# AlbertoEsc/PyFaceAnalysis

Measured on AMD Instinct MI355X. Metric: 128x128 sub-images/sec through 11L HiGSFA net, higher is better.
Workload: dtype f32; 1 GPU; configs[1]: U11L-128 (11-layer net, trained random-init weights), 4096 synthetic 128x128 sub-images per GPU per step, float32 input resident in HBM, first 20 slow features out; rows_per_gpu=4096, global_rows=4096, plan=fused, parallelism=row-shard x1

## Files before the change

### pyfaceanalysis_amd/build.py

```python
from __future__ import annotations

import os
import subprocess
import sys

HERE = os.path.dirname(os.path.abspath(__file__))
CSRC = os.path.join(HERE, "csrc")
LIB = os.path.join(HERE, "libhigsfa.so")
SOURCES = ["hg_tree.cpp", "hg_capi.cpp", "hg_hostpack.cpp", "hg_resample.cpp", "hg_normalize.cpp", "hg_normalize.hip", "hg_generic.hip", "hg_fused_plan.cpp", "hg_fused_call.cpp", "hg_fused.hip", "hg_fused_sum.hip", "hg_fused_front.hip", "hg_fused_igsfa.hip", "hg_fused_prod.hip", "hg_fused_tail.hip",
           "hg_gauss.hip", "hg_extract.hip", "hg_resample.hip", "hg_cascade.hip", "hg_eyes.hip", "hg_estimate.hip", "hg_train.hip"]
HEADERS = ["hg_common.hpp", os.path.join("..", "..", "include", "higsfa.h")]
HOST_ONLY = {"hg_hostpack.cpp": [], "hg_resample.cpp": ["-ffp-contract=off"], "hg_normalize.cpp": ["-ffp-contract=off"]}
HIPCC = os.environ.get("HIPCC", "/opt/rocm/bin/hipcc")
CXX = os.environ.get("CXX", "g++")
FLAGS = ["-O3", "-std=c++17", "-fPIC", "--offload-arch=gfx950", "-Wall", "-Wno-unused-result"]
if os.environ.get("HIGSFA_CXXFLAGS"):
    FLAGS += os.environ["HIGSFA_CXXFLAGS"].split()
if os.environ.get("HIGSFA_DIAG"):
    FLAGS.append("-DHIGSFA_DIAG")


def _newer(a, b):
    return (not os.path.exists(b)) or os.path.getmtime(a) > os.path.getmtime(b)


def _header_paths():
    hdr = [os.path.join(CSRC, h) for h in HEADERS]
    return hdr + [os.path.join(CSRC, h) for h in os.listdir(CSRC) if h.endswith((".hpp", ".h", ".inc"))]


def is_stale():
    if not os.path.exists(LIB):
        return True
    hdr = _header_paths()
    for src in SOURCES:
        sp, op = os.path.join(CSRC, src), os.path.join(CSRC, "_obj", src + ".o")
        if _newer(sp, op) or any(_newer(h, op) for h in hdr) or _newer(op, LIB):
            return True
    return False


def oracle_is_stale(oracle_dir):
    pairs = (("ref_c.c", "libref_c.so"), ("fast_cpu.c", "libfast_cpu.so"), ("fast_cpu_pow.c", "libfast_cpu.so"))
    return any(os.path.exists(os.path.join(oracle_dir, c)) and _newer(os.path.join(oracle_dir, c), os.path.join(oracle_dir, so))
               for c, so in pairs)


def build(force=False, verbose=False):
    objdir = os.path.join(CSRC, "_obj")
    os.makedirs(objdir, exist_ok=True)
    hdr_paths = [os.path.join(CSRC, h) for h in HEADERS]
    hdr_paths += [os.path.join(CSRC, h) for h in os.listdir(CSRC) if h.endswith((".hpp", ".h", ".inc"))]
    objs, relink = [], force or not os.path.exists(LIB)
    procs = []
    for src in SOURCES:
        sp = os.path.join(CSRC, src)
        op = os.path.join(objdir, src + ".o")
        objs.append(op)
        if force or _newer(sp, op) or any(_newer(h, op) for h in hdr_paths):
            if src in HOST_ONLY:
                cmd = [CXX, "-O3", "-std=c++17", "-fPIC", "-Wall"] + HOST_ONLY[src] + ["-c", sp, "-o", op]
            else:
                cmd = [HIPCC] + FLAGS + (["-x", "hip"] if src.endswith(".hip") else []) + ["-c", sp, "-o", op]
            if verbose:
                print(" ".join(cmd), flush=True)
            procs.append((src, subprocess.Popen(cmd, stdout=subprocess.PIPE, stderr=subprocess.STDOUT)))
            relink = True
    for src, p in procs:
        out, _ = p.communicate()
        if p.returncode != 0:
            raise RuntimeError("hipcc failed on %s:\n%s" % (src, out.decode(errors="replace")))
        if verbose and out:
            print(out.decode(errors="replace"))
    if relink:
        cmd = [HIPCC, "-shared", "-fPIC", "--offload-arch=gfx950", "-o", LIB] + objs + ["-L/opt/rocm/lib", "-lrocsolver", "-lrocblas"]
        if verbose:
            print(" ".join(cmd), flush=True)
        r = subprocess.run(cmd, stdout=subprocess.PIPE, stderr=subprocess.STDOUT)
        if r.returncode != 0:
            raise RuntimeError("link failed:\n%s" % r.stdout.decode(errors="replace"))
    return LIB


if __name__ == "__main__":
    print(build(force="--force" in sys.argv, verbose=True))
```

### pyfaceanalysis_amd/csrc/hg_fused.hip

```cpp
#include <hip/hip_runtime.h>

#include <algorithm>
#include <cmath>
#include <cstdlib>
#include <map>
#include <sstream>
#include <tuple>

#include "hg_fused_dev.hpp"

namespace hg {

namespace {

using namespace fused;

#ifndef HG_A_PINGPONG
#define HG_A_PINGPONG 1
#endif
#ifdef HIGSFA_DIAG
#define HG_HOT(blk) ((P.whatif & 1) ? ((blk) & 1) : (blk))
#else
#define HG_HOT(blk) (blk)
#endif
// ... 374 lines not shown
                            }
                    }
                }
            }
        }
        if (rem1) {
#pragma unroll
            for (int t = 0; t < T; ++t) add_rem4(z[t], d4[t]);
        }
        if (!P.has_exp) {
#pragma unroll
            for (int t = 0; t < T; ++t)
                if (tile[t] < P.n_tiles) P.out[((size_t)tile[t] * P.nb_out + node * P.mto + w) * 64 + lane] = z[t];
            return;
        }
        for (int fi = 0; fi < nf; ++fi) {
            const int fk = (P.funcp >> (4 * fi)) & 15;
            const float ex = P.expo[fi];
#pragma unroll
            for (int t = 0; t < T; ++t) smem[((fi * mt1n + w) * T + t) * 64 + lane] = apply_func_uniform(fk, ex, z[t]);
        }
    } else if (!P.has_exp) {
        return;
    }
    __syncthreads();
    if (w >= mt2n) return;
#pragma unroll
    for (int t = 0; t < T; ++t) d4[t] = f32x4{0.f, 0.f, 0.f, 0.f};
    f32x4 y[T];
    {
        const f32x4 bb = *(const f32x4*)(bnode + (mt1n + w) * 16);
#pragma unroll
        for (int t = 0; t < T; ++t) y[t] = bb;
    }
#pragma unroll
    for (int k = 0; k < KB; ++k) {
        if (k >= k2n) continue;
        const int mt1 = k / nf, fi = k - mt1 * nf;
        const int nk = (P.nk2p[mt1] >> (4 * fi)) & 15;
        f32x4 e[T];
#pragma unroll
        for (int t = 0; t < T; ++t) e[t] = smem[((fi * mt1n + mt1) * T + t) * 64 + lane];
        if (REM && rem2) {
#pragma unroll
            for (int r = 0; r < 4; ++r)
                if (r < nk) {
#pragma unroll
                    for (int t = 0; t < T; ++t) d4[t] = MFMA4(a2[k][r], e[t][r], d4[t]);
                }
        } else if (nk == 4) {
#pragma unroll
            for (int r = 0; r < 4; ++r)
#pragma unroll
                for (int t = 0; t < T; ++t) y[t] = MFMA16(a2[k][r], e[t][r], y[t]);
        } else {
#pragma unroll
            for (int r = 0; r < 4; ++r)
                if (r < nk) {
#pragma unroll
                    for (int t = 0; t < T; ++t) y[t] = MFMA16(a2[k][r], e[t][r], y[t]);
                }
        }
    }
    if (rem2) {
#pragma unroll
        for (int t = 0; t < T; ++t) add_rem4(y[t], d4[t]);
    }
    if (REM && P.pack_base > 0) {
        if (rem2) {
            const int slot = __builtin_amdgcn_readfirstlane(P.pack_slot[node]);
#pragma unroll
            for (int t = 0; t < T; ++t)
                if (tile[t] < P.n_tiles) *packed_slot_ptr(P, tile[t], slot, lane) = y[t][0];
        } else {
#pragma unroll
            for (int t = 0; t < T; ++t)
                if (tile[t] < P.n_tiles) P.out[((size_t)tile[t] * P.nb_out + node * (mt2n - 1) + w) * 64 + lane] = y[t];
        }
        return;
    }
#pragma unroll
    for (int t = 0; t < T; ++t)
        if (tile[t] < P.n_tiles) P.out[((size_t)tile[t] * P.nb_out + node * P.mto + w) * 64 + lane] = y[t];
}

template <typename YT>
__global__ void k_unpack(const float* __restrict__ act, int nb, const int32_t* __restrict__ col_base, YT* __restrict__ y,
                         int64_t ldy, int64_t n, int cols) {
    int64_t total = n * cols;
    for (int64_t idx = (int64_t)blockIdx.x * blockDim.x + threadIdx.x; idx < total; idx += (int64_t)gridDim.x * blockDim.x) {
        int64_t row = idx / cols;
        int c = (int)(idx - row * cols);
        int64_t tile = row >> 4;
        int jj = (int)(row & 15);
        y[row * ldy + c] = (YT)act[tile * nb * 256 + col_base[c] + jj * 4];
    }
}


template <int MT1, int MT2>
StageFn pick_stage_t(int T) {
    if (T == 2) return k_stage<MT1, MT2, 2>;
    return k_stage<MT1, MT2, 1>;
}
template <int MT1>
StageFn pick_stage_m2(int mt2, int T) {
    switch (mt2) {
        case 1: return pick_stage_t<MT1, 1>(T);
        case 2: return pick_stage_t<MT1, 2>(T);
        case 3: return pick_stage_t<MT1, 3>(T);
        default: return pick_stage_t<MT1, 4>(T);
    }
}
StageFn pick_stage(int mt1, int mt2, int T, bool rem = false, int kbf = 0, bool fs = false, int pk = -1) {
    if (pk >= 0) {
        if (pk == 1 && kbf == 3 && T == 2 && rem && mt1 == 3 && mt2 == 3) return fs ? (StageFn)k_stage<3, 3, 2, false, true, 3, true, 1> : (StageFn)k_stage<3, 3, 2, false, true, 3, false, 1>;
        if (pk == 1 && kbf == 3 && T == 2 && rem && mt1 == 2 && mt2 == 2) return (StageFn)k_stage<2, 2, 2, false, true, 3, false, 1>;
        return nullptr;
    }
    if (fs) {
        if (kbf == 3 && T == 2 && rem && mt1 == 3 && mt2 == 3) return (StageFn)k_stage<3, 3, 2, false, true, 3, true>;
        if (kbf == 4 && T == 2 && !rem && mt1 == 3 && mt2 == 3) return (StageFn)k_stage<3, 3, 2, false, false, 4, true>;
        if (kbf == 0 && !rem && mt1 == 4 && mt2 == 4) return T == 2 ? (StageFn)k_stage<4, 4, 2, false, false, 0, true> : (StageFn)k_stage<4, 4, 1, false, false, 0, true>;
    }
    if (kbf == 4 && T == 2) {
        if (rem && mt1 == 3 && mt2 == 3) return (StageFn)k_stage<3, 3, 2, false, true, 4>;
        if (rem && mt1 == 2 && mt2 == 2) return (StageFn)k_stage<2, 2, 2, false, true, 4>;
        if (!rem && mt1 == 3 && mt2 == 3) return (StageFn)k_stage<3, 3, 2, false, false, 4>;
        if (!rem && mt1 == 2 && mt2 == 2) return (StageFn)k_stage<2, 2, 2, false, false, 4>;
    }
    if (kbf == 3 && T == 2) {
        if (rem && mt1 == 3 && mt2 == 3) return (StageFn)k_stage<3, 3, 2, false, true, 3>;
        if (rem && mt1 == 2 && mt2 == 2) return (StageFn)k_stage<2, 2, 2, false, true, 3>;
    }
    if (rem) {
        if (mt1 == 3 && mt2 == 3) return T == 2 ? (StageFn)k_stage<3, 3, 2, false, true> : (StageFn)k_stage<3, 3, 1, false, true>;
        if (mt1 == 2 && mt2 == 2) return T == 2 ? (StageFn)k_stage<2, 2, 2, false, true> : (StageFn)k_stage<2, 2, 1, false, true>;
    }
    switch (mt1) {
        case 1: return pick_stage_m2<1>(mt2, T);
        case 2: return pick_stage_m2<2>(mt2, T);
        case 3: return pick_stage_m2<3>(mt2, T);
        default: return pick_stage_m2<4>(mt2, T);
    }
}



struct StageDev {
    DevBuf afrag, bias, kb1tab, chunks, runs, piece, koff, kmean, kcol, gcol, etab, pack_slot;
    DevBuf fold_frag, fold_bias;
    DevBuf fold_last;
    DevBuf pair_kids, kb1tab_pre, bias_pre;
};
struct SubRunDev {
    DevBuf nodes[kMaxTail], tab[kMaxTail];
};

struct WorkQueue {
    DevBuf ctr;
    uint32_t base = 0;
};

constexpr int kMaxLanes = 2;
struct Lane {
    DevBuf bufA, bufB;
    int64_t cap_rows = 0;
    WorkQueue wq_front, wq_direct, wq_direct_wg;
    int32_t* err_host = nullptr;
    int32_t* err_dev = nullptr;
    std::vector<CallStep> steps;
};

class FusedExecutor : public Executor {
public:
    explicit FusedExecutor(std::unique_ptr<const FusedPlan> plan) : plan_(std::move(plan)) {}

    int plan_kind() const override { return HG_PLAN_FUSED; }
    int n_stages() const override { return (int)plan_->stages.size() + 1; }
    std::string stage_name(int i) const override {
        if (i == 1 && plan_->fuse01 && !plan_->opt.fold01)
            return plan_->stages[i].name + "  [link 0 -> 1 stays as it is: switched off (HIGSFA_NO_FOLD01)]";
        if (i == 1 && plan_->fold01 && !plan_->opt.fold01_pack)
            return plan_->stages[i].name + "  [the link's one-row k-steps stay as they are: switched off (HIGSFA_NO_FOLD01_PACK)]";
        if (i < (int)plan_->stages.size() && plan_->stages[i].sum_in && !plan_->opt.pair)
            return plan_->stages[i].name + "; unpaired: switched off (HIGSFA_NO_PAIR)";
        if (i < (int)plan_->stages.size()) return plan_->stages[i].name;
        return plan_->tail_begin >= 0 ? std::string("row-major y written by the top-of-hierarchy launch (no unpack pass)")
                                      : std::string("fused unpack (fragment order -> row-major y)");
    }
    std::string describe() const override {
        std::ostringstream os;
        os << "plan: FUSED (fragment-order activations, v_mfma_f32_16x16x4_f32)\n";
        for (int i = 0; i < n_stages(); ++i) os << "  [" << i << "] " << stage_name(i) << "\n";
        return os.str();
    }
    int64_t weight_bytes() const override {
        int64_t t = 0;
        for (auto& s : plan_->stages) t += (int64_t)(s.afrag.size() + s.bias.size()) * 4;
        return t;
    }
    int64_t padded_flops_per_row() const override { return plan_->padded_flops_given; }
    int64_t workspace_bytes() const override {
        int64_t t = 0;
        for (int l = 0; l < n_lanes_; ++l) t += (int64_t)(lanes_[l].bufA.bytes + lanes_[l].bufB.bytes);
        return t;
    }

    void to_device() override {
        dev_.resize(plan_->stages.size());
        for (size_t si = 0; si < dev_.size(); ++si) {
            const HostStage& s = plan_->stages[si];
            StageDev& d = dev_[si];
            if (plan_->fold01 && si < 2) {
                const size_t first = si == 0 ? 0 : (size_t)s.kb1 * s.mt1, count = si == 0 ? (size_t)s.kb1 * s.mt1 : (size_t)s.node_blocks - first;
                std::vector<float> part((size_t)s.n_nodes * count * 256);
                for (int ni = 0; ni < s.n_nodes; ++ni)
                    std::copy_n(s.afrag.data() + ((size_t)ni * s.node_blocks + first) * 256, count * 256, part.data() + (size_t)ni * count * 256);
                const bool variant = plan_->fold01_pack && si == 0;
                if (variant) d.afrag.upload(s.fold_a1.data(), s.fold_a1.size() * 4);
                else d.afrag.upload(part.data(), part.size() * 4);
                if (si == 1) {
                    d.fold_frag.upload(s.fold_frag.data(), s.fold_frag.size() * 4);
                    d.fold_bias.upload(s.fold_bias.data(), s.fold_bias.size() * 4);
                    if (plan_->fold01_pack) d.fold_last.upload(s.fold_last.data(), s.fold_last.size() * 4);
                }
            } else {
                d.afrag.upload(s.afrag.data(), s.afrag.size() * 4);
            }
            if (plan_->fold01_pack && si == 0) d.bias.upload(s.fold_b1.data(), s.fold_b1.size() * 4);
            else d.bias.upload(s.bias.data(), s.bias.size() * 4);
            if (!s.kb1tab.empty()) d.kb1tab.upload(s.kb1tab.data(), s.kb1tab.size() * 4);
            if (!s.gcol.empty()) d.gcol.upload(s.gcol.data(), s.gcol.size() * 4);
            if (!s.etab.empty()) d.etab.upload(s.etab.data(), s.etab.size() * 4);
            if (!s.pack_slot.empty()) d.pack_slot.upload(s.pack_slot.data(), s.pack_slot.size() * 4);
            if (!s.pair_kids.empty()) {
                d.pair_kids.upload(s.pair_kids.data(), s.pair_kids.size() * 4);
                d.kb1tab_pre.upload(s.kb1tab_pre.data(), s.kb1tab_pre.size() * 4);
                d.bias_pre.upload(s.bias_pre.data(), s.bias_pre.size() * 4);
            }
            if (!s.chunks.empty()) {
                d.chunks.upload(s.chunks.data(), s.chunks.size() * sizeof(DChunk));
                d.runs.upload(s.runs.data(), s.runs.size() * sizeof(DRun));
                d.piece.upload(s.piece_col.data(), s.piece_col.size() * 4);
                d.koff.upload(s.koff.data(), s.koff.size() * 4);
                d.kmean.upload(s.kmean.data(), s.kmean.size() * 4);
                if (!s.kcol.empty()) d.kcol.upload(s.kcol.data(), s.kcol.size() * 4);
            }
        }
        sub_dev_.resize(plan_->sub_runs.size());
        for (size_t ri = 0; ri < sub_dev_.size(); ++ri) {
            const SubRun& r = plan_->sub_runs[ri];
            for (int k = 0; k < r.len; ++k) {
                sub_dev_[ri].nodes[k].upload(r.nodes[k].data(), r.nodes[k].size() * 4);
                if (k > 0) sub_dev_[ri].tab[k].upload(r.tab[k].data(), r.tab[k].size() * 4);
            }
        }
        d_col_base_.upload(plan_->col_base.data(), plan_->col_base.size() * 4);
        d_col_of_.upload(plan_->col_of.data(), plan_->col_of.size() * 4);
        int dev = 0;
        hipDeviceProp_t prop;
        if (hipGetDevice(&dev) == hipSuccess && hipGetDeviceProperties(&prop, dev) == hipSuccess && prop.multiProcessorCount > 0)
            n_cus_ = prop.multiProcessorCount;
    }

    void reserve(int64_t rows) override {
        for (int l = 0; l < n_lanes_; ++l) reserve_lane(lanes_[l], rows);
    }

    bool set_lanes(int n) override {
        if (n < 1 || n > kMaxLanes) return false;
        for (int l = n; l < n_lanes_; ++l) release_lane(lanes_[l]);
        for (int l = n_lanes_; l < n; ++l) reserve_lane(lanes_[l], lanes_[0].cap_rows);
        n_lanes_ = n;
        return true;
    }
    int lanes() const override { return n_lanes_; }

    void run(const void* x, int x_dtype, int64_t n, int64_t ldx, void* y, int y_dtype, int64_t y_cols, int64_t ldy,
             hipStream_t st, hipEvent_t* ev) override {
        run_in(lanes_[0], x, x_dtype, n, ldx, y, y_dtype, y_cols, ldy, st, ev);
    }
    void run_lane(int lane, const void* x, int x_dtype, int64_t n, int64_t ldx, void* y, int y_dtype, int64_t y_cols, int64_t ldy,
                  hipStream_t st) override {
        if (lane < 0 || lane >= n_lanes_) fail(HG_ERR_ARG, "lane %d outside 0..%d", lane, n_lanes_ - 1);
        run_in(lanes_[lane], x, x_dtype, n, ldx, y, y_dtype, y_cols, ldy, st, nullptr);
    }

    void run_in(Lane& L, const void* x, int x_dtype, int64_t n, int64_t ldx, void* y, int y_dtype, int64_t y_cols, int64_t ldy,
                hipStream_t st, hipEvent_t* ev) {
        check_device_error();
        if (dev_.size() != plan_->stages.size()) fail(HG_ERR_STATE, "fused: the plan is not on a device");
        if (n > L.cap_rows) {
            if (n_lanes_ > 1) HG_HIP(hipStreamSynchronize(st));
            reserve_lane(L, n);
        }
        run_range(L, x, x_dtype, n, ldx, y, y_dtype, y_cols, ldy, st, ev);
    }

    void run_range(Lane& L, const void* x, int x_dtype, int64_t n, int64_t ldx, void* y, int y_dtype, int64_t y_cols, int64_t ldy,
                   hipStream_t st, hipEvent_t* ev) {
        const int n_tiles = (int)((n + 15) / 16);
        FrontInput fi;
        fi.vec4_ok = rows_vec4(x, ldx, x_dtype);
        fi.x_dtype = x_dtype;
        fi.ldx = ldx;
        plan_call(*plan_, n_tiles, fi, L.steps);
        int e = 0;
        auto record = [&](int k) {
            if (ev)
                for (int i = 0; i < k; ++i) HG_HIP(hipEventRecord(ev[e++], st));
        };
        record(1);
        f32x4* cur = (f32x4*)L.bufA.p;
        f32x4* nxt = (f32x4*)L.bufB.p;
        for (const CallStep& step : L.steps) {
            const int si = step.stage;
            if (step.route == Route::Top) {
                debug_line(step, 0, 1);
                launch_top(si, cur, n_tiles, y, y_dtype, y_cols, ldy, n, st);
                record(step.covered + 1);
                HG_HIP(hipGetLastError());
                return;
            }
            if (step.route == Route::Subtree) {
                debug_line(step, 0, 1);
                launch_subtrees(plan_->sub_runs[step.sub_run], sub_dev_[step.sub_run], cur, nxt, n_tiles, st);
                std::swap(cur, nxt);
                record(step.covered);
                continue;
            }
            const HostStage& s = plan_->stages[si];
            const StageDev& d = dev_[si];
            StageParams P = stage_params(s, d, cur, nxt, n_tiles);
            switch (step.route) {
                case Route::Gather:
                    debug_line(step, 0, 1);
                    launch_im2frag(x, x_dtype, ldx, n, n_tiles, s.nb_out, (const int32_t*)d.gcol.p, nxt, step.sh.vec4 ? 1 : 0, (unsigned)step_blocks(step, 1), st);
                    break;
                case Route::IgSweep:
                case Route::IgSplit: launch_igsfa(step, s, P, st); break;
                case Route::Front01d:
                case Route::Front01p: launch_front_pair(L, step, s, d, P, x, x_dtype, ldx, n, n_tiles, cur, st); break;
                case Route::Front0p:
                case Route::Front0: launch_front(step, s, d, P, x, x_dtype, ldx, n, st); break;
                case Route::ProdSweep: launch_prod(step, s, d, P, st); break;
                case Route::Splitm: launch_splitm(step, s, P, st); break;
                default:
                    if (step.in_summed) {
                        P.kb1tab = (const int2*)d.kb1tab_pre.p;
                        P.bias = (const float*)d.bias_pre.p;
                        P.kb1 = step.sh.kb1;
                        P.n_kids = step.sh.n_kids;
                        P.nb_in = s.n_nodes * s.mt1;
                    }
                    if (step.route == Route::SumPair) launch_stage_pair(step, s, plan_->stages[si + 1], dev_[si + 1], P, st);
                    else launch_stage(step, s, P, st);
            }
            if (step.covered == 1) std::swap(cur, nxt);
            record(step.covered);
        }
        launch_unpack(cur, n, y, y_dtype, y_cols, ldy, st);
        record(1);
        HG_HIP(hipGetLastError());
    }

    void release() override {
        for (Lane& L : lanes_) release_lane(L);
        n_lanes_ = 1;
        d_col_base_.free();
        d_col_of_.free();
        sub_dev_.clear();
        dev_.clear();
    }

private:
    void reserve_lane(Lane& L, int64_t rows) {
        int64_t tiles = (rows + 15) / 16;
        size_t need = (size_t)tiles * plan_->max_nb * 1024;
        L.bufA.alloc(need);
        L.bufB.alloc(need);
        L.cap_rows = std::max(L.cap_rows, tiles * 16);
        L.steps.reserve(plan_->stages.size());
    }
    void release_lane(Lane& L) {
        L.bufA.free();
        L.bufB.free();
        L.wq_front.ctr.free();
        L.wq_direct.ctr.free();
        L.wq_direct_wg.ctr.free();
        L.wq_front.base = L.wq_direct.base = L.wq_direct_wg.base = 0;
        if (L.err_host) (void)hipHostFree(L.err_host);
        L.err_host = nullptr;
        L.err_dev = nullptr;
        L.cap_rows = 0;
    }

    int resident_blocks(StageFn fn, int threads, size_t lds) {
        set_lds_limit(fn, lds);
        auto key = std::make_tuple((const void*)fn, threads, lds);
        auto it = occ_.find(key);
        if (it != occ_.end()) return it->second;
        int nb = 0;
        if (hipOccupancyMaxActiveBlocksPerMultiprocessor(&nb, (const void*)fn, threads, lds) != hipSuccess || nb < 1) nb = 1;
        occ_[key] = nb;
        return nb;
    }

    uint32_t* work_counters(WorkQueue& q, int n, hipStream_t st) {
        const size_t need = (size_t)n * 64;
        if (q.ctr.bytes < need) {
            q.ctr.alloc(std::max<size_t>(need, 64 * 1024));
            HG_HIP(hipMemsetD32Async((hipDeviceptr_t)q.ctr.p, (int)plan_->opt.wq_start, q.ctr.bytes / 4, st));
            q.base = plan_->opt.wq_start;
        }
        return (uint32_t*)q.ctr.p;
    }

    int32_t* device_error_word(Lane& L) {
        if (!L.err_host) {
            HG_HIP(hipHostMalloc((void**)&L.err_host, 64, hipHostMallocMapped));
            *L.err_host = 0;
            HG_HIP(hipHostGetDevicePointer((void**)&L.err_dev, L.err_host, 0));
        }
        return L.err_dev;
    }
    void check_errors() override { check_device_error(); }
    void check_device_error() {
        for (const Lane& L : lanes_)
            if (L.err_host && *(volatile int32_t*)L.err_host != 0)
                fail(HG_ERR_DEVICE, "fused: a bounded poll in a persistent kernel ran out (code %d); the features of that call are invalid", (int)*L.err_host);
    }

    void set_lds_limit(StageFn fn, size_t bytes) {
        if (bytes <= 64 * 1024) return;
        if (bytes > 160 * 1024) fail(HG_ERR_FORMAT, "fused: a node needs %zu bytes of LDS (> 160 KiB)", bytes);
        auto it = lds_set_.find((const void*)fn);
        if (it != lds_set_.end() && it->second >= bytes) return;
        HG_HIP(hipFuncSetAttribute((const void*)fn, hipFuncAttributeMaxDynamicSharedMemorySize, (int)(160 * 1024)));
        lds_set_[(const void*)fn] = 160 * 1024;
    }

    StageParams stage_params(const HostStage& hs, const StageDev& d, const f32x4* in, f32x4* out, int n_tiles) const {
        StageParams R{};
        R.afrag = (const f32x4*)d.afrag.p;
        R.bias = (const float*)d.bias.p;
        R.kb1tab = (const int2*)d.kb1tab.p;
        R.in = in;
        R.out = out;
        R.n_nodes = hs.n_nodes;
        R.kb1 = hs.kb1;
        R.nf = hs.nf;
        R.has_exp = hs.has_exp ? 1 : 0;
        R.node_blocks = hs.node_blocks;
        R.bias_floats = hs.bias_floats;
        R.n_tiles = n_tiles;
        R.nb_in = hs.nb_in;
        R.nb_out = hs.nb_out;
        R.mto = hs.mto;
        R.pack_base = hs.pack_out ? hs.n_nodes * (hs.mto - 1) : 0;
        R.pack_soa = hs.pack_soa ? 1 : 0;
        R.pack_in = hs.pack_in;
        R.pack_slot = (const int32_t*)d.pack_slot.p;
        R.a4x4 = hs.rem4 ? 1 : 0;
        R.sum_in = hs.sum_in ? 1 : 0;
        R.n_kids = hs.n_kids;
        if (plan_->fold01 && (&hs == &plan_->stages[0] || &hs == &plan_->stages[1])) {
            const bool first = &hs == &plan_->stages[0];
            R.node_blocks = first ? hs.kb1 * hs.mt1 : hs.node_blocks - hs.kb1 * hs.mt1;
            R.fold_frag = (const f32x4*)d.fold_frag.p;
            R.fold_bias = (const float*)d.fold_bias.p;
            R.fold_last = (const float*)d.fold_last.p;
            if (plan_->fold01_pack && first) R.bias_floats = 16;
        }
        for (int fi = 0; fi < hs.nf; ++fi) {
            R.funcp |= (uint32_t)hs.funcs[fi].kind << (4 * fi);
            R.expo[fi] = (float)hs.funcs[fi].expo;
            for (int mt1 = 0; mt1 < hs.mt1; ++mt1) R.nk2p[mt1] |= (uint32_t)hs.nk2[mt1][fi] << (4 * fi);
        }
        return R;
    }

    static bool rows_vec4(const void* x, int64_t ldx, int x_dtype) {
        const size_t esz = dtype_size(x_dtype), valign = x_dtype == HG_U8 ? 4 : 16;
        return ldx % 4 == 0 && ((uintptr_t)x % valign) == 0 && (ldx * esz) % valign == 0;
    }

    int64_t fill_sweep(const CallStep& step, StageFn fn, StageParams& P) {
        const CallShape& sh = step.sh;
        const int occ = resident_blocks(fn, sh.threads, sh.lds);
        P.nodes_per_group = sh.per_group;
        P.nodes_per_wg = sh.per_group;
        P.n_chunks = sh.n_groups;
        P.tile_groups = sh.tile_groups;
        P.tile_parts = step_tile_parts(step, occ);
        debug_line(step, occ, P.tile_parts);
        return step_blocks(step, P.tile_parts);
    }

    void debug_line(const CallStep& step, int occ, int tile_parts) const {
// ... 11 lines not shown
#endif
        launch_tail(TP, T, st);
#ifdef HIGSFA_DIAG
        if (stamped) tail_stamps_report("top-of-hierarchy launch", si, TP.n_stages, (size_t)((n_tiles + T - 1) / T), st);
#endif
    }

    void launch_subtrees(const SubRun& sr, const SubRunDev& sd, const f32x4* in, f32x4* out, int n_tiles, hipStream_t st) {
        TailParams TP = subtree_params(sr, sd, in, out, n_tiles);
#ifdef HIGSFA_DIAG
        const bool stamped = plan_->opt.stamp_stage == sr.begin;
        if (stamped) tail_stamps_begin(TP, (size_t)sr.n * n_tiles, st);
#endif
        launch_subtree(TP, st);
#ifdef HIGSFA_DIAG
        if (stamped) tail_stamps_report("sub-tree launch", sr.begin, TP.n_stages, (size_t)sr.n * n_tiles, st);
#endif
    }

    void launch_igsfa(const CallStep& step, const HostStage& s, StageParams& P, hipStream_t st) {
        const CallShape& sh = step.sh;
        if (step.route == Route::IgSplit) {
            P.ig_folded = 1;
            debug_line(step, 0, 1);
            launch_igfold_split(P, s.mt2, sh.T, (unsigned)step_blocks(step, 1), sh.threads, sh.lds, st);
            return;
        }
        StageFn fn = s.ig_folded ? pick_igfold(s.mt2, sh.T, sh.fs) : pick_igsfa(s.mt1, s.mt2, sh.T, s.kb1);
        const int64_t blocks = fill_sweep(step, fn, P);
        P.nodes_per_wg = sh.nw;
        P.ig_has_lr = s.ig_has_lr ? 1 : 0;
        P.ig_folded = s.ig_folded ? 1 : 0;
        P.nk2p[0] = 0;
        for (int ms = 0; ms < s.mt1; ++ms) P.nk2p[0] |= (uint32_t)s.ig_nks[ms] << (4 * ms);
        hipLaunchKernelGGL(fn, (unsigned)blocks, sh.threads, sh.lds, st, P);
    }

    void front_params(const CallStep& step, const HostStage& s, const StageDev& d, StageParams& P, const void* x, int64_t ldx, int64_t n) const {
        P.chunks = (const DChunk*)d.chunks.p;
        P.runs = (const DRun*)d.runs.p;
        P.piece_col = (const int2*)d.piece.p;
        P.koff = (const int32_t*)d.koff.p;
        P.kmean = (const float*)d.kmean.p;
        P.kcol = (const int32_t*)d.kcol.p;
        P.x = x;
        P.ldx = ldx;
        P.n_rows = n;
        P.lds_stride = s.lds_stride;
        P.nk_last = s.nk_last;
        P.contig4 = s.contig4 ? 1 : 0;
        P.n_chunks = step.sh.n_groups;
        P.vec4 = step.sh.vec4 ? 1 : 0;
    }

    void launch_front_pair(Lane& L, const CallStep& step, const HostStage& s, const StageDev& d, StageParams& P, const void* x, int x_dtype, int64_t ldx, int64_t n,
                           int n_tiles, f32x4* out1, hipStream_t st) {
        const CallShape& sh = step.sh;
        const bool direct = step.route == Route::Front01d;
        front_params(step, s, d, P, x, ldx, n);
        StageParams Q = stage_params(plan_->stages[1], dev_[1], nullptr, out1, n_tiles);
        if (sh.pack && (!Q.fold_last || P.bias_floats != 16)) fail(HG_ERR_STATE, "internal: a packed plan without its packed fragments on the device");
        StageFn2 fn = direct ? pick_stage01d(x_dtype, false, sh.wgq, sh.fold, sh.pack) : pick_stage01p(x_dtype, false, sh.rem4, sh.fspec, sh.fold, sh.scalar, sh.pack);
        if (!fn) fail(HG_ERR_STATE, "internal: no packed front kernel for this plan");
        const int occ = resident_blocks((StageFn)fn, sh.threads, sh.lds);
        P.tile_parts = step_tile_parts(step, occ);
        debug_line(step, occ, P.tile_parts);
        const unsigned blocks = (unsigned)step_blocks(step, P.tile_parts);
#ifdef HIGSFA_DIAG
        if (plan_->opt.stamp_stage == 0 && x_dtype == HG_F32 && (direct || !sh.fold)) {
            fn = direct ? pick_stage01d(HG_F32, true, sh.wgq, sh.fold, sh.pack) : pick_stage01p(HG_F32, true, sh.rem4, sh.fspec, sh.fold);
            stamps_begin(P, (int)blocks, 12, st);
        }
#endif
        P.err = device_error_word(L);
        {
            WorkQueue& wq = direct ? (sh.wgq ? L.wq_direct_wg : L.wq_direct) : L.wq_front;
            P.work_ctr = work_counters(wq, sh.queue_ctrs, st);
            P.work_base = wq.base;
            wq.base += (uint32_t)sh.tile_groups;
        }
#ifdef HIGSFA_DIAG
        if (const char* e = getenv("HIGSFA_WHATIF")) P.whatif = atoi(e);
#endif
        hipLaunchKernelGGL(fn, blocks, sh.threads, sh.lds, st, P, Q);
#ifdef HIGSFA_DIAG
        if (P.stamps) front_stamps_report(P.n_chunks, st);
#endif
    }

    void launch_front(const CallStep& step, const HostStage& s, const StageDev& d, StageParams& P, const void* x, int x_dtype, int64_t ldx, int64_t n, hipStream_t st) {
        const CallShape& sh = step.sh;
        front_params(step, s, d, P, x, ldx, n);
        const bool persistent = step.route == Route::Front0p;
        StageFn fn = persistent ? pick_stage0p(x_dtype) : pick_stage0(s.mt1, s.mt2, sh.T, x_dtype);
        const int occ = persistent ? resident_blocks(fn, sh.threads, sh.lds) : 0;
        if (persistent) P.tile_parts = step_tile_parts(step, occ);
        const int64_t blocks = step_blocks(step, P.tile_parts);
        debug_line(step, occ, P.tile_parts);
        set_lds_limit(fn, sh.lds);
        hipLaunchKernelGGL(fn, (unsigned)blocks, sh.threads, sh.lds, st, P);
    }

    void launch_splitm(const CallStep& step, const HostStage& s, const StageParams& P, hipStream_t st) {
        const CallShape& sh = step.sh;
        const unsigned grid = (unsigned)step_blocks(step, 1);
        debug_line(step, 0, 1);
        if (sh.rem4) {
            if (sh.T == 2) hipLaunchKernelGGL((k_stage_splitm<2, true>), grid, sh.threads, sh.lds, st, P, s.mt1, s.mt2);
            else hipLaunchKernelGGL((k_stage_splitm<1, true>), grid, sh.threads, sh.lds, st, P, s.mt1, s.mt2);
        } else if (sh.T == 2)
            hipLaunchKernelGGL(k_stage_splitm<2>, grid, sh.threads, sh.lds, st, P, s.mt1, s.mt2);
        else
            hipLaunchKernelGGL(k_stage_splitm<1>, grid, sh.threads, sh.lds, st, P, s.mt1, s.mt2);
    }

    void launch_stage(const CallStep& step, const HostStage& s, StageParams& P, hipStream_t st) {
        const CallShape& sh = step.sh;
        StageFn fn = s.pk_kbi >= 0 ? (sh.kbf == 3 ? pick_stage(s.mt1, s.mt2, sh.T, s.rem4, sh.kbf, sh.fs, s.pk_kbi) : nullptr) : pick_stage(s.mt1, s.mt2, sh.T, s.rem4, sh.kbf, sh.fs);
        if (!fn) fn = pick_stage(s.mt1, s.mt2, sh.T, s.rem4, 0, false);
        if (s.sum_in) fn = pick_stage_sum(s.mt1, s.mt2, sh.T, sh.fs);
        const int64_t blocks = fill_sweep(step, fn, P);
        P.pair_chunks = sh.pair_chunks ? 1 : 0;
#ifdef HIGSFA_DIAG
        const int si = step.stage, T = sh.T, kbf = sh.kbf;
        const bool stamp_kbf3 = s.mt1 == 3 && s.mt2 == 3 && T == 2 && s.rem4 && kbf == 3;
        if (plan_->opt.stamp_stage == si && !s.sum_in && (stamp_kbf3 || (s.mt1 == s.mt2 && (s.mt1 == 4 || s.mt1 == 3) && T == 2 && !s.rem4 && kbf == 0))) {
            fn = stamp_kbf3 ? (StageFn)k_stage<3, 3, 2, true, true, 3> : s.mt1 == 4 ? (StageFn)k_stage<4, 4, 2, true> : (StageFn)k_stage<3, 3, 2, true>;
            stamps_begin(P, (int)blocks, 8, st);
        }
#endif
        set_lds_limit(fn, sh.lds);
#ifdef HIGSFA_DIAG
        if (const char* e = getenv("HIGSFA_WHATIF")) P.whatif = atoi(e);
#endif
        hipLaunchKernelGGL(fn, (unsigned)blocks, sh.threads, sh.lds, st, P);
#ifdef HIGSFA_DIAG
        if (P.stamps) stage_stamps_report(si, blocks, sh.nw, st);
#endif
    }

    void launch_stage_pair(const CallStep& step, const HostStage& s, const HostStage& parent, const StageDev& pd, StageParams& P, hipStream_t st) {
        const CallShape& sh = step.sh;
        StageFn fn = pick_stage_sum_pair(sh.T);
        if (!fn) fail(HG_ERR_STATE, "internal: no pair kernel of %d tiles per wave", sh.T);
        P.pair_kids = (const int2*)pd.pair_kids.p;
        P.pair_bias = (const float*)pd.bias.p;
        P.pair_bias_floats = parent.bias_floats;
        P.n_pairs = parent.n_nodes;
        P.nb_out = parent.n_nodes * s.mto;
        const int64_t blocks = fill_sweep(step, fn, P);
        hipLaunchKernelGGL(fn, (unsigned)blocks, sh.threads, sh.lds, st, P);
    }

    void launch_prod(const CallStep& step, const HostStage& s, const StageDev& d, StageParams& P, hipStream_t st) {
        StageFn fn = pick_prod(s.mt1, s.mt2, step.sh.T);
        const int64_t blocks = fill_sweep(step, fn, P);
        P.etab = (const int2*)d.etab.p;
        P.neb = s.neb;
        P.nk_last = s.nk_last;
        P.has_clip = s.has_clip ? 1 : 0;
        P.clip_lo = s.clip_lo;
        P.clip_hi = s.clip_hi;
        hipLaunchKernelGGL(fn, (unsigned)blocks, step.sh.threads, step.sh.lds, st, P);
    }

    void launch_unpack(const f32x4* in, int64_t n, void* y, int y_dtype, int64_t y_cols, int64_t ldy, hipStream_t st) {
        const HostStage& last = plan_->stages.back();
        unsigned grid = (unsigned)std::min<int64_t>((n * y_cols + 255) / 256, 4096);
        if (y_dtype == HG_F32)
            hipLaunchKernelGGL(k_unpack<float>, grid, 256, 0, st, (const float*)in, last.nb_out, (const int32_t*)d_col_base_.p,
                               (float*)y, ldy, n, (int)y_cols);
        else if (y_dtype == HG_F64)
            hipLaunchKernelGGL(k_unpack<double>, grid, 256, 0, st, (const float*)in, last.nb_out, (const int32_t*)d_col_base_.p,
                               (double*)y, ldy, n, (int)y_cols);
        else
            fail(HG_ERR_ARG, "output dtype must be f32 or f64");
    }

#ifdef HIGSFA_DIAG
    void tail_stamps_begin(TailParams& TP, size_t blocks, hipStream_t st) {
        stamp_buf_.alloc(blocks * 16 * 16 * 8);
        HG_HIP(hipMemsetAsync(stamp_buf_.p, 0, stamp_buf_.bytes, st));
        TP.stamps = (unsigned long long*)stamp_buf_.p;
    }
    void tail_stamps_report(const char* what, int si, int n_layers, size_t blocks, hipStream_t st) {
        HG_HIP(hipStreamSynchronize(st));
        std::vector<unsigned long long> h(blocks * 16 * 16);
        HG_HIP(hipMemcpy(h.data(), stamp_buf_.p, h.size() * 8, hipMemcpyDeviceToHost));
        unsigned long long t0 = ~0ull;
        for (size_t i = 0; i < h.size(); i += 16)
            if (h[i]) t0 = std::min(t0, h[i]);
        static const char* names[5] = {"loads in", "expanded", "barrier 1", "outputs stored", "barrier 2"};
        double sum[16] = {}, mx[16] = {}, cnt[16] = {};
        for (size_t i = 0; i < h.size(); i += 16)
            for (int k = 0; k < 16; ++k)
                if (h[i + k]) {
                    const double us = (double)(h[i + k] - t0) * 0.01;
                    sum[k] += us; cnt[k] += 1; mx[k] = std::max(mx[k], us);
                }
        fprintf(stderr, "[stamp stage %d] %s, %zu workgroups: us after the first wave's entry, mean (max) over the waves that took part\n", si, what, blocks);
        fprintf(stderr, "[stamp stage %d]   entry %.2f (%.2f)\n", si, cnt[0] ? sum[0] / cnt[0] : 0.0, mx[0]);
        for (int l = 0; l < n_layers; ++l) {
            fprintf(stderr, "[stamp stage %d]   layer %d:", si, l);
            for (int k = 0; k < 5; ++k) {
                const int q = 1 + 5 * l + k;
                fprintf(stderr, "  %s %.2f (%.2f; %.0f waves)", names[k], cnt[q] ? sum[q] / cnt[q] : 0.0, mx[q], cnt[q]);
            }
            fprintf(stderr, "\n");
        }
    }
    void stamps_begin(StageParams& P, int blocks, int words, hipStream_t st) {
        stamp_blocks_ = blocks;
        stamp_buf_.alloc((size_t)blocks * 8 * words * 8);
        HG_HIP(hipMemsetAsync(stamp_buf_.p, 0, stamp_buf_.bytes, st));
        P.stamps = (unsigned long long*)stamp_buf_.p;
    }
    void front_stamps_report(int n_chunks, hipStream_t st) {
        HG_HIP(hipStreamSynchronize(st));
        std::vector<unsigned long long> h((size_t)stamp_blocks_ * 8 * 12);
        HG_HIP(hipMemcpy(h.data(), stamp_buf_.p, h.size() * 8, hipMemcpyDeviceToHost));
        double a[7] = {0, 0, 0, 0, 0, 0, 0}, nwv = 0;
        unsigned long long lo[3] = {~0ull, ~0ull, ~0ull}, hi[3] = {0, 0, 0};
        for (size_t i = 0; i < h.size(); i += 12)
            if (h[i + 4]) {
                for (int k = 0; k < 7; ++k) a[k] += h[i + k];
                nwv += 1;
                for (int k = 0; k < 3; ++k) { lo[k] = std::min(lo[k], h[i + 7 + k]); hi[k] = std::max(hi[k], h[i + 7 + k]); }
            }
        {
            double xs[8][4] = {}, ps[16][3] = {};
            for (size_t i = 0, w = 0; i < h.size(); i += 12, ++w)
                if (h[i + 4]) {
                    const int blk = (int)(w / 8), xc = blk % 8, pt = std::min(15, blk / n_chunks);
                    const double life = (h[i + 9] - h[i + 8]) * 0.01, clk = (double)h[i + 4] / (double)h[i + 5] * 100.0;
                    xs[xc][0] += 1; xs[xc][1] += life; xs[xc][2] = std::max(xs[xc][2], life); xs[xc][3] += clk;
                    ps[pt][0] += 1; ps[pt][1] += life; ps[pt][2] = std::max(ps[pt][2], life);
                }
            for (int k = 0; k < 8; ++k)
                if (xs[k][0] > 0) fprintf(stderr, "[stamp stage 0+1] xcd %d: waves %.0f loop us mean %.1f max %.1f clock %.0f MHz\n", k, xs[k][0], xs[k][1] / xs[k][0], xs[k][2], xs[k][3] / xs[k][0]);
            for (int k = 0; k < 16; ++k)
                if (ps[k][0] > 0) fprintf(stderr, "[stamp stage 0+1] part %d: waves %.0f loop us mean %.1f max %.1f\n", k, ps[k][0], ps[k][1] / ps[k][0], ps[k][2]);
        }
        fprintf(stderr, "[stamp stage 0+1] wall clock, us after the first wave's entry: entries until %.1f, loop starts %.1f..%.1f, ends %.1f..%.1f\n",
                (hi[0] - lo[0]) * 0.01, (lo[1] - lo[0]) * 0.01, (hi[1] - lo[0]) * 0.01, (lo[2] - lo[0]) * 0.01, (hi[2] - lo[0]) * 0.01);
        fprintf(stderr, "[stamp stage 0+1] waves %.0f clock %.0f MHz lifetime %.1f us, iterations %.1f; cycles per iteration: "
                        "lds-write+barrier %.0f, fetch issue %.0f, layer0 %.0f, layer1+store %.0f (sum %.0f)\n",
                nwv, a[4] / a[5] * 100.0, a[5] / nwv / 100.0, a[6] / nwv, a[0] / a[6], a[1] / a[6], a[2] / a[6], a[3] / a[6],
                (a[0] + a[1] + a[2] + a[3]) / a[6]);
    }
    void stage_stamps_report(int si, int64_t blocks, int nw, hipStream_t st) {
        HG_HIP(hipStreamSynchronize(st));
        std::vector<unsigned long long> h((size_t)stamp_blocks_ * 8 * 8);
        HG_HIP(hipMemcpy(h.data(), stamp_buf_.p, h.size() * 8, hipMemcpyDeviceToHost));
        double c = 0, g1 = 0, tl = 0, all = 0, it = 0, nwv = 0, rt = 0;
        unsigned long long lo0 = ~0ull, hi0 = 0, lo1 = ~0ull, hi1 = 0;
        std::vector<unsigned long long> ends;
        for (size_t i = 0; i < h.size(); i += 8)
            if (h[i + 3]) {
                c += h[i]; g1 += h[i + 1]; tl += h[i + 2]; all += h[i + 3]; it += h[i + 4]; rt += h[i + 5]; nwv += 1;
                lo0 = std::min(lo0, h[i + 6]); hi0 = std::max(hi0, h[i + 6]); lo1 = std::min(lo1, h[i + 7]); hi1 = std::max(hi1, h[i + 7]);
                ends.push_back(h[i + 7]);
            }
        std::sort(ends.begin(), ends.end());
        if (!ends.empty())
            fprintf(stderr, "[stamp stage %d] wall clock, us after the first wave's start: starts until %.1f, ends %.1f (10%%) %.1f (50%%) %.1f (90%%) %.1f (last); grid %lld blocks x %d waves\n",
                    (int)si, (hi0 - lo0) * 0.01, (ends[ends.size() / 10] - lo0) * 0.01, (ends[ends.size() / 2] - lo0) * 0.01,
                    (ends[ends.size() * 9 / 10] - lo0) * 0.01, (hi1 - lo0) * 0.01, (long long)blocks, nw);
        fprintf(stderr, "[stamp stage %d] in-kernel clock %.0f MHz, wave lifetime %.1f us\n", (int)si, all / rt * 100.0, rt / nwv / 100.0);
        fprintf(stderr, "[stamp stage %d] waves %.0f  avg cycles/wave: total %.0f  copy+barrier %.0f  gemm1 %.0f  tail %.0f  node-iterations %.1f  (per iteration: gemm1 %.0f tail %.0f)\n",
                (int)si, nwv, all / nwv, c / nwv, g1 / nwv, tl / nwv, it / nwv, g1 / it, tl / it);
    }
#endif

    static void fill_tail_stage(TailStage& S, const HostStage& hs, const StageDev& d) {
        S.afrag = (const f32x4*)d.afrag.p;
        S.bias = (const float*)d.bias.p;
        S.kb1tab = (const int2*)d.kb1tab.p;
        S.n_nodes = hs.n_nodes;
        S.kb1 = hs.kb1;
        S.nf = hs.nf;
        S.has_exp = hs.has_exp ? 1 : 0;
        S.node_blocks = hs.node_blocks;
        S.bias_floats = hs.bias_floats;
        S.nb_out = hs.nb_out;
        S.mto = hs.mto;
        S.mt1 = hs.mt1;
        S.mt2 = hs.mt2;
        S.sum_in = hs.sum_in ? 1 : 0;
        S.n_kids = hs.n_kids;
        for (int fi = 0; fi < hs.nf; ++fi) {
            S.funcp |= (uint32_t)hs.funcs[fi].kind << (4 * fi);
            S.expo[fi] = (float)hs.funcs[fi].expo;
            for (int mt1 = 0; mt1 < hs.mt1; ++mt1) S.nk2p[mt1] |= (uint32_t)hs.nk2[mt1][fi] << (4 * fi);
        }
    }

    TailParams subtree_params(const SubRun& sr, const SubRunDev& sd, const f32x4* in, f32x4* out, int n_tiles) {
        const int sub_begin_ = sr.begin, sub_len_ = sr.len, sub_n_ = sr.n, sub_act_blocks_ = sr.act_blocks, sub_e_blocks_ = sr.e_blocks;
        TailParams TP{};
        TP.n_stages = sub_len_;
        for (int k = 0; k < sub_len_; ++k) {
            fill_tail_stage(TP.st[k], plan_->stages[sub_begin_ + k], dev_[sub_begin_ + k]);
            TP.st[k].n_nodes /= sub_n_;
            TP.sub_nodes[k] = (const int32_t*)sd.nodes[k].p;
            if (k > 0) TP.st[k].kb1tab = (const int2*)sd.tab[k].p;
        }
// ... 58 lines not shown
```

### pyfaceanalysis_amd/csrc/hg_fused_call.cpp

```cpp
#include "hg_fused_call.hpp"

#include <algorithm>
#include <cmath>
#include <cstdio>
#include <cstdlib>

namespace hg {
namespace fused {

FusedOptions executor_options() {
    FusedOptions opt = FusedOptions::from_env();
    opt.hoist = getenv("HIGSFA_NO_HOIST") == nullptr;
    opt.fold01 = getenv("HIGSFA_NO_FOLD01") == nullptr;
    opt.fold01_pack = opt.fold01 && getenv("HIGSFA_NO_FOLD01_PACK") == nullptr;
    opt.pair = opt.hoist && getenv("HIGSFA_NO_PAIR") == nullptr;
    return opt;
}

bool fs_expansion(const HostStage& s, const FusedOptions& opt) {
    return s.nf == 2 && s.funcs[0].kind == E_IDENTITY && s.funcs[1].kind == E_ABS_POW && !opt.no_fspec;
}

const char* route_name(Route r) {
    static const char* const names[] = {"gather", "front01d", "front01p", "front0p", "front0", "igsweep", "igsplit", "prod", "splitm", "sweep", "sumpair",
                                        "subtree", "top"};
    return names[(int)r];
}

namespace {

template <size_t N>
WavesTiles sweep_shape(const int (&cand)[N][2], int n_tiles, int n_groups) {
    WavesTiles sh{4, 1};
    for (auto& c : cand) {
        const int64_t tg = (n_tiles + c[0] * c[1] - 1) / (c[0] * c[1]);
        if (c[0] * c[1] <= n_tiles && tg * n_groups >= 256) {
            sh = {c[0], c[1]};
            break;
        }
    }
    while (sh.nw * sh.T > std::max(n_tiles, 1) && sh.nw > 1) sh.nw >>= 1;
    return sh;
}

int ceil_div(int a, int b) { return (a + b - 1) / b; }

int splitm_tiles(const HostStage& s, int n_tiles) { return n_tiles >= 2 * 256 / std::max(1, s.n_nodes) ? 2 : 1; }
bool splitm_takes(const HostStage& s, int n_tiles, const FusedOptions& opt) {
    const int64_t wgs = (int64_t)ceil_div(n_tiles, splitm_tiles(s, n_tiles)) * s.n_nodes;
    return s.kind == 0 && (!s.rem4 || s.mt1 == s.mt2) && (s.rem4 || !s.pack_out) && s.mt1 * s.nf <= 8 &&
           (s.n_nodes <= opt.splitm_max_nodes ? (int64_t)s.n_nodes * n_tiles <= 8192 : wgs <= opt.splitm_max_wgs);
}

bool igsplit_takes(const HostStage& s, int n_tiles) {
    return s.ig_folded && s.n_nodes <= 8 && s.nf <= 2 && s.kb1 <= 8 && (int64_t)s.n_nodes * n_tiles <= 16384;
}

int pair_group(const HostStage& s, const FusedOptions& opt) {
    const int kib = 2 * std::max(1, s.node_blocks);
    return std::max(1, std::min(opt.sum_lds_kib, kPairLdsCapKiB) / kib);
}
int pair_waves(int n_tiles) {
    int nw = 8;
    while (nw * kPairTiles > std::max(n_tiles, 1) && nw > 1) nw >>= 1;
    return nw;
}
bool link_summed(const HostStage& s, const HostStage& p, int n_tiles, bool in_summed, const FusedOptions& opt) {
    if (p.pair_kids.empty() || !s.sum_in || s.n_nodes != 2 * p.n_nodes) return false;
    if (!in_summed && (s.pair_kids.empty() || s.kb1 != 2 * s.mt1)) return false;
    if (!(s.has_exp && fs_expansion(s, opt)) || s.mt1 != 4 || s.mt2 != 4 || p.mt1 != 4 || s.mto != 4 || s.pack_out || s.rem4) return false;
    const int ppg = pair_group(s, opt), nw = pair_waves(n_tiles);
    const int64_t n_groups = (p.n_nodes + ppg - 1) / ppg, tile_groups = (n_tiles + nw * kPairTiles - 1) / (nw * kPairTiles);
    return n_groups * tile_groups >= opt.pair_min_wgs;
}

void shape_gather(const HostStage& s, int n_tiles, const FrontInput& fi, CallShape& sh) {
    sh.vec4 = s.vec_ok && fi.vec4_ok;
    sh.threads = 256;
    sh.blocks = ((int64_t)n_tiles * s.nb_out + 3) / 4;
}

Route shape_front(const FusedPlan& plan, int n_tiles, const FrontInput& fi, CallShape& sh) {
    const HostStage& s = plan.stages[0];
    const int chunks = (int)s.chunks.size();
    sh.vec4 = s.vec_ok && fi.vec4_ok;
    sh.n_groups = chunks;
    if (plan.fuse01) {
        const HostStage& s1 = plan.stages[1];
        sh.rem4 = s1.rem4 || (s1.p_max <= 20 && s1.s_max <= 20 && s1.nk2[1][0] <= 1 && s1.nk2[1][1] <= 1 && !plan.opt.no_rem4);
        sh.fspec = fs_expansion(s, plan.opt) && fs_expansion(s1, plan.opt);
    }
    const int FT = stage01p_tiles(sh.rem4, sh.fspec);
    sh.fold = plan.fold01;
    if (sh.fold && !(sh.rem4 && plan.fuse01)) fail(HG_ERR_STATE, "internal: the link 0 -> 1 is folded but the front kernel's remainder-tile form does not apply");
    sh.pack = plan.fold01_pack;
    if (sh.pack && !sh.fold) fail(HG_ERR_STATE, "internal: packed k-steps on a plan whose link 0 -> 1 is not folded");
    if (plan.fuse01 && ((sh.vec4 && n_tiles >= FT) || sh.fold)) {
        const HostStage& s1 = plan.stages[1];
        sh.direct = sh.vec4 && sh.fspec && sh.rem4 && s.direct_ok && s1.pack_out && (int64_t)16 * fi.ldx * (int64_t)dtype_size(fi.x_dtype) + 2048 < 0x7fffffffll &&
                    s.max_chunk_nodes <= 8 && !plan.opt.no_direct;
        sh.wgq = !plan.opt.no_wgq;
        sh.scalar = sh.fold && !sh.vec4;
        sh.T = FT;
        sh.threads = 64 * std::max(1, (s.max_chunk_nodes + 1) / 2);
        sh.lds = sh.direct ? (size_t)4 * 160 * 4 + 32 * 4 + (size_t)4 * 256 * 4
                           : (size_t)(kDoubleBuffer01 ? 2 : 1) * FT * 16 * s.lds_stride * 4 + (size_t)(sh.threads / 64) * 160 * 4 + 16;
        sh.tile_groups = ceil_div(n_tiles, FT);
        sh.queue_ctrs = sh.direct && !sh.wgq ? s1.n_nodes : chunks;
        return sh.direct ? Route::Front01d : Route::Front01p;
    }
    if (sh.fold) fail(HG_ERR_STATE, "internal: an unfused first-layer kernel on a plan whose link 0 -> 1 is folded");
    sh.T = (n_tiles >= 4 && s.mt1 * s.mt2 <= 4) ? 4 : 1;
    sh.tile_groups = ceil_div(n_tiles, sh.T);
    sh.lds = (size_t)sh.T * 16 * s.lds_stride * 4;
    const bool persistent = sh.T == 4 && sh.vec4 && s.contig4 && s.has_exp && s.mt1 == 1 && s.mt2 == 1 && s.kb1 == 1 && s.nf <= 2 && s.max_chunk_nodes <= 16 &&
                    64 * s.max_chunk_pieces <= 8 * 512;
    if (persistent) {
        sh.threads = 512;
        return Route::Front0p;
    }
    sh.threads = sh.T == 4 ? 512 : 256;
    sh.blocks = (int64_t)sh.tile_groups * chunks;
    return Route::Front0;
}

Route shape_igsfa(const HostStage& s, int n_tiles, const FusedOptions& opt, CallShape& sh) {
    if (igsplit_takes(s, n_tiles)) {
        sh.T = n_tiles >= 2 ? 2 : 1;
        sh.tile_groups = ceil_div(n_tiles, sh.T);
        sh.nw = std::max(s.kb1, s.mt2);
        sh.threads = sh.nw * 64;
        sh.lds = (size_t)s.nf * s.kb1 * sh.T * 1024;
        sh.blocks = (int64_t)sh.tile_groups * s.n_nodes;
        return Route::IgSplit;
    }
    int nwt = 1, T = 1;
    static const int cand[][2] = {{12, 2}, {8, 2}, {4, 2}};
    for (auto& c : cand) {
        if (c[0] == 12 && (s.ig_folded || !(s.kb1 == 5 || s.kb1 == 6))) continue;
        const int64_t tg = (n_tiles + c[0] * c[1] - 1) / (c[0] * c[1]);
        if (c[0] * c[1] <= std::max(n_tiles, 1) && tg * s.n_nodes >= 256) {
            nwt = c[0];
            T = c[1];
            break;
        }
    }
    if (nwt == 1 && T == 1) {
        T = n_tiles >= 2 ? 2 : 1;
        nwt = n_tiles >= 8 ? 4 : n_tiles >= 4 ? 2 : 1;
    }
    sh.nw = nwt;
    sh.T = T;
    sh.fs = s.ig_folded && fs_expansion(s, opt);
    sh.threads = std::max(nwt, 4) * 64;
    sh.lds = (size_t)s.node_blocks * 1024 + (size_t)s.bias_floats * 4 + (size_t)s.kb1 * 8;
    sh.tile_groups = ceil_div(n_tiles, nwt * T);
    sh.per_group = 1;
    sh.n_groups = s.n_nodes;
    return Route::IgSweep;
}

void shape_prod(const HostStage& s, int n_tiles, CallShape& sh) {
    static const int shapes[][2] = {{8, 2}, {4, 2}, {4, 1}};
    const WavesTiles wt = sweep_shape(shapes, n_tiles, s.n_nodes);
    const size_t zs_bytes = (size_t)wt.nw * wt.T * s.mt1 * 1024, et_bytes = (size_t)s.neb * 128;
    const size_t per_node = (size_t)s.node_blocks * 1024 + (size_t)s.bias_floats * 4 + (size_t)s.kb1 * 8;
    const size_t fixed = zs_bytes + et_bytes;
    sh.nw = wt.nw;
    sh.T = wt.T;
    sh.per_group = (int)std::max<size_t>(1, std::min<size_t>(s.n_nodes, fixed + per_node <= (size_t)kProdLdsBytes ? (kProdLdsBytes - fixed) / per_node : 1));
    sh.n_groups = ceil_div(s.n_nodes, sh.per_group);
    sh.tile_groups = ceil_div(n_tiles, wt.nw * wt.T);
    sh.threads = wt.nw * 64;
    sh.lds = (size_t)sh.per_group * per_node + et_bytes + zs_bytes;
}

void shape_splitm(const HostStage& s, int n_tiles, CallShape& sh) {
    sh.T = splitm_tiles(s, n_tiles);
    sh.tile_groups = ceil_div(n_tiles, sh.T);
    sh.nw = std::max(s.mt1, s.has_exp ? s.mt2 : 1);
    sh.threads = sh.nw * 64;
    sh.lds = (size_t)std::max(1, s.nf) * s.mt1 * sh.T * 1024;
    sh.rem4 = s.rem4;
    sh.blocks = (int64_t)sh.tile_groups * s.n_nodes;
}

void first_affine_read(const HostStage& s, bool in_summed, CallShape& sh) {
    sh.kb1 = in_summed ? s.mt1 : s.kb1;
    sh.n_kids = in_summed ? 1 : s.n_kids;
}

void shape_sweep(const HostStage& s, int n_tiles, bool in_summed, const FusedOptions& opt, CallShape& sh) {
    const int npg = std::max(1, std::min(s.n_nodes, (s.sum_in ? opt.sum_lds_kib : kWeightLdsKiB) / std::max(1, s.node_blocks)));
    const int n_groups = ceil_div(s.n_nodes, npg);
    const WavesTiles wt = stage_sweep_shape(n_tiles, n_groups);
    first_affine_read(s, in_summed, sh);
    sh.nw = wt.nw;
    sh.T = wt.T;
    sh.per_group = npg;
    sh.n_groups = n_groups;
    sh.tile_groups = ceil_div(n_tiles, wt.nw * wt.T);
    sh.threads = wt.nw * 64;
    sh.lds = (size_t)npg * s.node_blocks * 1024 + (size_t)npg * s.bias_floats * 4 + (size_t)npg * s.kb1 * 8;
    sh.kbf = (wt.T == 2 && s.mt1 == s.mt2 && (s.mt1 == 2 || s.mt1 == 3)) ? (s.kb1 == 4 ? 4 : (s.kb1 == 3 && s.rem4 ? 3 : 0)) : 0;
    sh.fs = s.has_exp && fs_expansion(s, opt);
    sh.rem4 = s.rem4;
    sh.pair_chunks = s.pack_out && !s.pack_soa && npg == 2 && n_groups % 16 == 0;
}

void shape_sum_pair(const HostStage& s, const HostStage& parent, int n_tiles, bool in_summed, const FusedOptions& opt, CallShape& sh) {
    const int ppg = std::min(pair_group(s, opt), parent.n_nodes);
    first_affine_read(s, in_summed, sh);
    sh.nw = pair_waves(n_tiles);
    sh.T = kPairTiles;
    sh.per_group = ppg;
    sh.n_groups = ceil_div(parent.n_nodes, ppg);
    sh.tile_groups = ceil_div(n_tiles, sh.nw * sh.T);
    sh.threads = sh.nw * 64;
    sh.lds = (size_t)2 * ppg * ((size_t)s.node_blocks * 1024 + (size_t)s.bias_floats * 4 + (size_t)sh.kb1 * 8) + (size_t)ppg * 256;
    sh.fs = true;
}

}

WavesTiles stage_sweep_shape(int n_tiles, int n_groups) {
    static const int shapes[][2] = {{8, 2}, {8, 1}, {4, 2}, {4, 1}};
    return sweep_shape(shapes, n_tiles, n_groups);
}

void plan_call(const FusedPlan& plan, int n_tiles, const FrontInput& fi, std::vector<CallStep>& steps) {
    steps.clear();
    const int ns = (int)plan.stages.size();
    const int sub_set = plan.pick_sub_set(n_tiles);
    const int top = plan.tail_begin >= 0 ? plan.tail_start(n_tiles) : ns;
    for (int si = 0; si < ns;) {
        CallStep st;
        st.stage = si;
        const HostStage& s = plan.stages[si];
        if (si == top) {
            st.route = Route::Top;
            st.covered = ns - si;
        } else {
            for (size_t ri = 0; ri < plan.sub_runs.size(); ++ri) {
                const SubRun& r = plan.sub_runs[ri];
                if (r.begin == si && r.set == sub_set && plan.sub_run_pays(r, n_tiles)) st.sub_run = (int)ri;
            }
            if (st.sub_run >= 0) {
                const SubRun& r = plan.sub_runs[st.sub_run];
                st.route = Route::Subtree;
                st.covered = r.len;
                st.sh.blocks = (int64_t)r.n * n_tiles;
            } else if (s.kind == 1) {
                st.route = Route::Gather;
                shape_gather(s, n_tiles, fi, st.sh);
            } else if (s.kind == 2) {
                st.route = shape_igsfa(s, n_tiles, plan.opt, st.sh);
            } else if (s.from_x) {
                st.route = shape_front(plan, n_tiles, fi, st.sh);
                if (st.route == Route::Front01d || st.route == Route::Front01p) st.covered = 2;
            } else if (s.kind == 3) {
                st.route = Route::ProdSweep;
                shape_prod(s, n_tiles, st.sh);
            } else if (splitm_takes(s, n_tiles, plan.opt)) {
                st.route = Route::Splitm;
                shape_splitm(s, n_tiles, st.sh);
            } else {
                st.route = Route::Sweep;
            }
        }
        steps.push_back(st);
        si += st.covered;
    }
    for (size_t i = 0; i < steps.size(); ++i) {
        CallStep& st = steps[i];
        if (st.route != Route::Sweep) continue;
        const HostStage& s = plan.stages[st.stage];
        if (i + 1 < steps.size() && steps[i + 1].route == Route::Sweep && link_summed(s, plan.stages[st.stage + 1], n_tiles, st.in_summed, plan.opt)) {
            st.route = Route::SumPair;
            steps[i + 1].in_summed = true;
            shape_sum_pair(s, plan.stages[st.stage + 1], n_tiles, st.in_summed, plan.opt, st.sh);
        } else {
            shape_sweep(s, n_tiles, st.in_summed, plan.opt, st.sh);
        }
    }
}

int sweep_tile_parts(int n_groups, int tile_groups, int occ) {
    const double capacity = 256.0 * occ;
    const int64_t g8 = (int64_t)(n_groups + 7) / 8 * 8;
    int tile_parts = 1;
    double best = 1e300;
    for (int pp = 1; pp <= tile_groups; ++pp) {
        const double rounds = std::ceil(g8 * pp / capacity);
        const double cost = rounds * (0.35 + (double)((tile_groups + pp - 1) / pp));
        if (cost < best - 1e-9) {
            best = cost;
            tile_parts = pp;
        }
    }
    return tile_parts;
}

int spread_tile_parts(int groups, int chunks, int occ) { return std::max(1, std::min(groups, 256 * occ / std::max(1, chunks))); }

int step_tile_parts(const CallStep& st, int occ) {
    switch (st.route) {
        case Route::Sweep:
        case Route::SumPair:
        case Route::ProdSweep: return sweep_tile_parts(st.sh.n_groups, st.sh.tile_groups, occ);
        case Route::IgSweep:
        case Route::Front01d:
        case Route::Front01p:
        case Route::Front0p: return spread_tile_parts(st.sh.tile_groups, st.sh.n_groups, occ);
        default: return 1;
    }
}

int64_t step_blocks(const CallStep& st, int tile_parts) {
    switch (st.route) {
        case Route::Sweep:
        case Route::SumPair:
        case Route::ProdSweep: {
            const int64_t blocks = (int64_t)((st.sh.n_groups + 7) / 8) * 8 * tile_parts;
            if (blocks > 0x7fffffffll) fail(HG_ERR_ARG, "batch too large");
            return blocks;
        }
        case Route::IgSweep:
        case Route::Front01d:
        case Route::Front01p:
        case Route::Front0p: return (int64_t)st.sh.n_groups * tile_parts;
        case Route::Front0:
            if (st.sh.blocks > 0x7fffffffll) fail(HG_ERR_ARG, "batch too large");
            return st.sh.blocks;
        default: return st.sh.blocks;
    }
}

const char* format_step(const FusedPlan& plan, const CallStep& st, int occ, int tile_parts, char* buf, size_t cap) {
    const HostStage& s = plan.stages[st.stage];
    const CallShape& sh = st.sh;
    const int si = st.stage;
    const long long blocks = st.route == Route::Top ? 0 : (long long)step_blocks(st, tile_parts);
    switch (st.route) {
        case Route::Gather:
            snprintf(buf, cap, "[gather stage %d] blocks_out %d vec4 %d threads %d blocks %lld", si, s.nb_out, (int)sh.vec4, sh.threads, blocks);
            break;
        case Route::Front01d:
        case Route::Front01p:
            snprintf(buf, cap, "[front] occ %d threads %d lds %zu chunks %d tile_parts %d", occ, sh.threads, sh.lds, sh.n_groups, tile_parts);
            break;
        case Route::Front0p:
        case Route::Front0:
            snprintf(buf, cap, "[front0] persistent %d tiles %d vec4 %d occ %d threads %d lds %zu chunks %d tile_groups %d tile_parts %d blocks %lld", (int)(st.route == Route::Front0p), sh.T,
                     (int)sh.vec4, occ, sh.threads, sh.lds, sh.n_groups, sh.tile_groups, tile_parts, blocks);
            break;
        case Route::IgSweep:
            snprintf(buf, cap, "[igsfa stage %d] nodes %d kb1 %d shape %dx%d occ %d lds %zu tile_groups %d parts %d", si, s.n_nodes, s.kb1, sh.nw, sh.T, occ, sh.lds,
                     sh.tile_groups, tile_parts);
            break;
        case Route::IgSplit:
            snprintf(buf, cap, "[igsplit stage %d] nodes %d mo %d kb1 %d tiles %d waves %d lds %zu blocks %lld", si, s.n_nodes, s.mt2, s.kb1, sh.T, sh.nw, sh.lds, blocks);
            break;
        case Route::ProdSweep:
            snprintf(buf, cap, "[prod stage %d] nodes %d mt1 %d mt2 %d neb %d shape %dx%d npg %d node_groups %d tile_groups %d parts %d", si, s.n_nodes, s.mt1, s.mt2, s.neb,
                     sh.nw, sh.T, sh.per_group, sh.n_groups, sh.tile_groups, tile_parts);
            break;
        case Route::Splitm:
            snprintf(buf, cap, "[splitm stage %d] nodes %d mt1 %d mt2 %d rem4 %d tiles %d waves %d lds %zu blocks %lld", si, s.n_nodes, s.mt1, s.mt2, (int)sh.rem4, sh.T, sh.nw,
                     sh.lds, blocks);
            break;
        case Route::Sweep:
            snprintf(buf, cap, "[sweep stage %d] nodes %d mt1 %d mt2 %d kb1 %d shape %dx%d npg %d node_groups %d tile_groups %d parts %d occ %d lds %zu kbf %d fs %d rem4 %d pk %d "
                     "hoisted %d summed_in %d pair_chunks %d", si, s.n_nodes, s.mt1, s.mt2, sh.kb1, sh.nw, sh.T, sh.per_group, sh.n_groups, sh.tile_groups, tile_parts, occ,
                     sh.lds, sh.kbf, (int)sh.fs, (int)sh.rem4, s.pk_kbi, (int)s.sum_in, (int)st.in_summed, (int)sh.pair_chunks);
            break;
        case Route::SumPair:
            snprintf(buf, cap, "[pair stage %d] pairs %d per group %d shape %dx%d lds %zu tile_groups %d parts %d kids in %d", si, plan.stages[si + 1].n_nodes, sh.per_group,
                     sh.nw, sh.T, sh.lds, sh.tile_groups, tile_parts, sh.n_kids);
            break;
        case Route::Subtree: {
            const SubRun& r = plan.sub_runs[st.sub_run];
            snprintf(buf, cap, "[subtree stage %d] layers %d subtrees %d set %d blocks %lld", si, r.len, r.n, r.set, blocks);
            break;
        }
        case Route::Top:
            snprintf(buf, cap, "[top stage %d] layers %d", si, st.covered);
            break;
    }
    return buf;
}

}
}
```

### pyfaceanalysis_amd/csrc/hg_fused_call.hpp

```cpp
#pragma once
#include <vector>

#include "hg_fused_plan.hpp"

namespace hg {
namespace fused {

constexpr int kWeightLdsKiB = 64;
constexpr int kProdLdsBytes = 52 * 1024;
constexpr int kPairLdsCapKiB = 144;
constexpr int kPairTiles = 1;
constexpr bool kDoubleBuffer01 = true;
constexpr int stage01p_tiles(bool , bool fspec) { return fspec ? 1 : 2; }

FusedOptions executor_options();

bool fs_expansion(const HostStage& s, const FusedOptions& opt);

enum class Route : uint8_t {
    Gather,
    Front01d,
    Front01p,
    Front0p,
    Front0,
    IgSweep,
    IgSplit,
    ProdSweep,
    Splitm,
    Sweep,
    SumPair,
    Subtree,
    Top,
};
const char* route_name(Route r);

struct FrontInput {
    bool vec4_ok = true;
    int x_dtype = HG_F32;
    int64_t ldx = 0;
};

struct CallShape {
    int nw = 0, T = 0;
    int per_group = 0;
    int n_groups = 0;
    int tile_groups = 0;
    int threads = 0;
    size_t lds = 0;
    int kbf = 0;
    bool fs = false;
    bool rem4 = false, fspec = false, direct = false, wgq = false, fold = false, pack = false, scalar = false;
    bool vec4 = false;
    bool pair_chunks = false;
    int kb1 = 0, n_kids = 0;
    int queue_ctrs = 0;
    int64_t blocks = 0;
};

struct CallStep {
    Route route = Route::Sweep;
    int stage = 0, covered = 1;
    bool in_summed = false;
    int sub_run = -1;
    CallShape sh;
};

void plan_call(const FusedPlan& plan, int n_tiles, const FrontInput& fi, std::vector<CallStep>& steps);

struct WavesTiles {
    int nw, T;
};
WavesTiles stage_sweep_shape(int n_tiles, int n_groups);

int sweep_tile_parts(int n_groups, int tile_groups, int occ);
int spread_tile_parts(int groups, int chunks, int occ);
int step_tile_parts(const CallStep& st, int occ);
int64_t step_blocks(const CallStep& st, int tile_parts);

const char* format_step(const FusedPlan& plan, const CallStep& st, int occ, int tile_parts, char* buf, size_t cap);

}
}
```

### pyfaceanalysis_amd/csrc/hg_fused_dev.hpp

```cpp
#pragma once
#include <hip/hip_runtime.h>

#include <algorithm>

#include "hg_fused_call.hpp"

namespace hg {
namespace fused {

typedef float f32x4 __attribute__((ext_vector_type(4)));
typedef int i32x4 __attribute__((ext_vector_type(4)));

struct StageParams {
    const f32x4* afrag;
    const float* bias;
    const int2* kb1tab;
    const f32x4* in;
    f32x4* out;
    int32_t n_nodes, kb1, nf, has_exp;
    int32_t node_blocks, bias_floats, n_tiles, nb_in, nb_out, mto;
    int32_t nodes_per_group, nodes_per_wg, n_chunks, tile_groups, tile_parts;
    uint32_t nk2p[kMaxMT];
    uint32_t funcp;
    float expo[kMaxFuncs];
// ... 232 lines not shown
                if (DUP || tile[t] < P.n_tiles) P.out[((size_t)tile[t] * P.nb_out + out_blk + mt) * 64 + lane] = z[mt][t];
        return;
    }
    f32x4 y[MT2][T];
#pragma unroll
    for (int mt = 0; mt < MT2; ++mt) {
        f32x4 bb = *(const f32x4*)(b2 + mt * 16 + g * 4);
#pragma unroll
        for (int t = 0; t < T; ++t) y[mt][t] = bb;
    }
    const float ex0 = P.expo[0], ex1 = P.expo[1], ex2 = P.expo[2], ex3 = P.expo[3];
    const uint32_t funcp = P.funcp;
    const int nf = P.nf;
    f32x4 d4[T];
#pragma unroll
    for (int t = 0; t < T; ++t) d4[t] = f32x4{0.f, 0.f, 0.f, 0.f};
    if constexpr (FS) {
#pragma unroll
        for (int mt1 = 0; mt1 < MT1; ++mt1) {
            const uint32_t nkp = P.nk2p[mt1];
            const int nk0 = nkp & 15, nk1 = (nkp >> 4) & 15;
            if constexpr (REM) {
                gemm_block_rem<MT2, T>(wA2 + (mt1 * 2) * MT2 * 64, z[mt1], y, d4, nk0);
                f32x4 e[T];
#pragma unroll
                for (int t = 0; t < T; ++t) e[t] = pow_abs4(z[mt1][t], ex1);
                gemm_block_rem<MT2, T>(wA2 + (mt1 * 2 + 1) * MT2 * 64, e, y, d4, nk1);
            } else if constexpr (LEAN) {
                gemm_block<MT2, T>(wA2 + (mt1 * 2) * MT2 * 64, z[mt1], y, nk0);
                f32x4 e[T];
#pragma unroll
                for (int t = 0; t < T; ++t) e[t] = pow_abs4(z[mt1][t], ex1);
                gemm_block<MT2, T>(wA2 + (mt1 * 2 + 1) * MT2 * 64, e, y, nk1);
            } else if constexpr (!HG_POW_PREFETCH) {
                gemm_block<MT2, T, true>(wA2 + (mt1 * 2) * MT2 * 64, z[mt1], y, nk0);
                f32x4 e[T];
#pragma unroll
                for (int t = 0; t < T; ++t) e[t] = pow_abs4(z[mt1][t], ex1);
                gemm_block<MT2, T, true>(wA2 + (mt1 * 2 + 1) * MT2 * 64, e, y, nk1);
            } else {
                gemm_block<MT2, T, true>(wA2 + (mt1 * 2) * MT2 * 64, z[mt1], y, nk0);
                f32x4 ap[MT2];
#pragma unroll
                for (int mt = 0; mt < MT2; ++mt) ap[mt] = (wA2 + (mt1 * 2 + 1) * MT2 * 64)[mt * 64];
                f32x4 e[T];
#pragma unroll
                for (int t = 0; t < T; ++t) e[t] = pow_abs4(z[mt1][t], ex1);
                gemm_block_regs<MT2, T>(ap, e, y, nk1);
            }
        }
    } else
#pragma unroll
    for (int mt1 = 0; mt1 < MT1; ++mt1) {
        const uint32_t nkp = P.nk2p[mt1];
        for (int fi = 0; fi < nf; ++fi) {
            const int nk = (nkp >> (4 * fi)) & 15;
            if (nk == 0) continue;
            f32x4 e[T];
            const int fk = (funcp >> (4 * fi)) & 15;
            const float ex = fi == 0 ? ex0 : (fi == 1 ? ex1 : (fi == 2 ? ex2 : ex3));
#pragma unroll
            for (int t = 0; t < T; ++t) e[t] = apply_func(fk, ex, z[mt1][t]);
            if constexpr (REM) gemm_block_rem<MT2, T>(wA2 + (mt1 * nf + fi) * MT2 * 64, e, y, d4, nk);
            else gemm_block<MT2, T>(wA2 + (mt1 * nf + fi) * MT2 * 64, e, y, nk);
        }
    }
    if constexpr (REM) {
#pragma unroll
        for (int t = 0; t < T; ++t) {
            if (rscr) y[MT2 - 1][t][0] += rem4_total_lds(d4[t], rscr, lane);
            else add_rem4(y[MT2 - 1][t], d4[t]);
        }
        if constexpr (DUP) {
            const bool packed = P.pack_base > 0;
            const int blk0 = packed ? node * (MT2 - 1) : out_blk;
#pragma unroll
            for (int mt = 0; mt < MT2 - 1; ++mt)
#pragma unroll
                for (int t = 0; t < T; ++t)
                    if (!no_store) P.out[((size_t)tile[t] * P.nb_out + blk0 + mt) * 64 + lane] = y[mt][t];
            if (packed) {
#pragma unroll
                for (int t = 0; t < T; ++t)
                    if (!no_store) *packed_slot_ptr(P, tile[t], slot_in, lane) = y[MT2 - 1][t][0];
            } else {
#pragma unroll
                for (int t = 0; t < T; ++t)
                    if (!no_store) P.out[((size_t)tile[t] * P.nb_out + out_blk + MT2 - 1) * 64 + lane] = y[MT2 - 1][t];
            }
            return;
        } else if (P.pack_base > 0) {
#pragma unroll
            for (int mt = 0; mt < MT2 - 1; ++mt)
#pragma unroll
                for (int t = 0; t < T; ++t)
                    if (tile[t] < P.n_tiles && !no_store) P.out[((size_t)tile[t] * P.nb_out + node * (MT2 - 1) + mt) * 64 + lane] = y[mt][t];
            const int slot = __builtin_amdgcn_readfirstlane(P.pack_slot[node]);
#pragma unroll
            for (int t = 0; t < T; ++t)
                if (tile[t] < P.n_tiles && !no_store)
                    *packed_slot_ptr(P, tile[t], slot, lane) = y[MT2 - 1][t][0];
            return;
        }
    }
#pragma unroll
    for (int mt = 0; mt < MT2; ++mt)
#pragma unroll
        for (int t = 0; t < T; ++t)
            if ((DUP || tile[t] < P.n_tiles) && !no_store) P.out[((size_t)tile[t] * P.nb_out + out_blk + mt) * 64 + lane] = y[mt][t];
}


struct TailStage {
    const f32x4* afrag;
    const float* bias;
    const int2* kb1tab;
    int32_t n_nodes, kb1, nf, has_exp, node_blocks, bias_floats, nb_out, mto, mt1, mt2;
    int32_t sum_in, n_kids;
    uint32_t nk2p[kMaxMT], funcp;
    float expo[kMaxFuncs];
};
struct TailParams {
    TailStage st[kMaxTail];
    const f32x4* in;
    void* y;
    const int32_t* col_of;
    int64_t ldy, n_rows;
    int32_t y_cols, y_f64;
    int32_t n_stages, n_tiles, nb_in;
    int32_t act_blocks, e_blocks;
    f32x4* out_frag;
    const int32_t* sub_nodes[kMaxTail];
    int32_t n_sub, nb_out_frag;
    unsigned long long* stamps;
};
size_t tail_lds_bytes(const TailParams& P, int T);
int tail_waves(const TailParams& P);
void launch_tail(const TailParams& P, int T, hipStream_t st);
void launch_subtree(const TailParams& P, hipStream_t st);


typedef void (*StageFn)(StageParams);
typedef void (*StageFn2)(StageParams, StageParams);

StageFn pick_stage0(int mt1, int mt2, int T, int x_dtype);
StageFn pick_stage0p(int x_dtype);
StageFn2 pick_stage01p(int x_dtype, bool stamp, bool rem4, bool fspec, bool fold = false, bool scalar = false, bool pack = false);
StageFn2 pick_stage01d(int x_dtype, bool stamp, bool wgq, bool fold = false, bool pack = false);
StageFn pick_igsfa(int ms, int mo, int T, int kb1);
StageFn pick_igfold(int mo, int T, bool fs = false);
StageFn pick_prod(int mt1, int mt2, int T);
StageFn pick_stage_sum(int mt1, int mt2, int T, bool fs);
StageFn pick_stage_sum_pair(int T);
void launch_igfold_split(const StageParams& P, int mo, int T, unsigned grid, int threads, size_t lds, hipStream_t st);
void launch_im2frag(const void* x, int x_dtype, int64_t ldx, int64_t n_rows, int n_tiles, int nb, const int32_t* gcol, f32x4* out,
                    int vec4, unsigned grid, hipStream_t st);

template <typename XT> struct Vec4Load;
typedef uint32_t u32x4_t __attribute__((ext_vector_type(4)));
constexpr int kBufferFlags = 0x00020000;
template <> struct Vec4Load<float> {
    static __device__ __forceinline__ f32x4 ld(const float* p) { return *(const f32x4*)p; }
    static __device__ __forceinline__ f32x4 buf(__amdgpu_buffer_rsrc_t r, uint32_t off) {
        return __builtin_bit_cast(f32x4, __builtin_amdgcn_raw_buffer_load_b128(r, off, 0, 0));
    }
};
template <> struct Vec4Load<uint8_t> {
    static __device__ __forceinline__ f32x4 ld(const uint8_t* p) {
        uint32_t w = *(const uint32_t*)p;
        f32x4 v;
        v[0] = (float)(w & 0xff);
        v[1] = (float)((w >> 8) & 0xff);
        v[2] = (float)((w >> 16) & 0xff);
        v[3] = (float)(w >> 24);
        return v;
    }
    static __device__ __forceinline__ f32x4 buf(__amdgpu_buffer_rsrc_t r, uint32_t off) {
        const uint32_t w = __builtin_amdgcn_raw_buffer_load_b32(r, off, 0, 0);
        return f32x4{(float)(w & 0xff), (float)((w >> 8) & 0xff), (float)((w >> 16) & 0xff), (float)(w >> 24)};
    }
};
template <> struct Vec4Load<double> {
    static __device__ __forceinline__ f32x4 ld(const double* p) {
        typedef double f64x2 __attribute__((ext_vector_type(2)));
        f64x2 a = *(const f64x2*)p, b = *(const f64x2*)(p + 2);
        f32x4 v;
        v[0] = (float)a[0];
        v[1] = (float)a[1];
        v[2] = (float)b[0];
        v[3] = (float)b[1];
        return v;
    }
    static __device__ __forceinline__ f32x4 buf(__amdgpu_buffer_rsrc_t r, uint32_t off) {
        typedef double f64x2 __attribute__((ext_vector_type(2)));
        const f64x2 a = __builtin_bit_cast(f64x2, __builtin_amdgcn_raw_buffer_load_b128(r, off, 0, 0));
        const f64x2 b = __builtin_bit_cast(f64x2, __builtin_amdgcn_raw_buffer_load_b128(r, off + 16, 0, 0));
        return f32x4{(float)a[0], (float)a[1], (float)b[0], (float)b[1]};
    }
};


}
}
```

### pyfaceanalysis_amd/csrc/hg_fused_plan.cpp

```cpp
#include <algorithm>
#include <cmath>
#include <map>
#include <sstream>
#include <tuple>

#include "hg_fused_plan.hpp"
#include "hg_fused_stages.hpp"

namespace hg {
namespace fused {

namespace {

Aff aff_of(const TNode& n) { return Aff{(int)n.in_dim, (int)n.out_dim, n.a, n.W, n.b}; }

Aff fold(const Aff& f, const Aff& s) {
    Aff r;
    r.in = f.in;
    r.out = s.out;
    r.a = f.a;
    r.W.assign((size_t)f.in * s.out, 0.0);
    for (int i = 0; i < f.in; ++i)
        for (int k = 0; k < f.out; ++k) {
            double w = f.W[(size_t)i * f.out + k];
// ... 250 lines not shown
            continue;
        }
        if (c.kind == K_IDENTITY) continue;
        std::vector<ChainT> chains;
        if (!to_chains(c, chains, why)) return false;
        bool merged = false;
        if (!group.empty() && group.size() == chains.size()) {
            merged = true;
            for (size_t k = 0; k < chains.size(); ++k)
                if (group[k].out_dim != chains[k].in_dim) { merged = false; break; }
            if (merged)
                for (size_t k = 0; k < chains.size() && merged; ++k) {
                    int n_exp = 0, n_ig = 0;
                    for (auto* l : group[k].seq) { n_exp += l->kind == K_EXPANSION; n_ig += l->kind == K_IGSFA; }
                    for (auto* l : chains[k].seq) { n_exp += l->kind == K_EXPANSION; n_ig += l->kind == K_IGSFA; }
                    if (n_exp > 1 || n_ig > 0) merged = false;
                }
            if (merged)
                for (size_t k = 0; k < chains.size(); ++k) {
                    group[k].out_dim = chains[k].out_dim;
                    for (auto* l : chains[k].seq) group[k].seq.push_back(l);
                }
        }
        if (!merged) {
            if (!close_group()) return false;
            group = std::move(chains);
        }
    }
    if (!close_group()) return false;
    if (have_pending) { why = "flow ends in a switchboard"; return false; }
    if (stages.empty()) { why = "no layer in the flow"; return false; }
    return true;
}

namespace {
struct LinkFold {
    std::vector<double> bias;
    std::vector<std::vector<double>> W;
};
LinkFold fold_link(const FStage& ch, const FStage& pa, int pj, const std::vector<int>& owner, const std::vector<int>& col0, const std::vector<int>& kids) {
    const FNode& pn = pa.nodes[pj];
    const int P = pn.A1.out;
    LinkFold lf;
    lf.bias = pn.A1.b;
    lf.W.resize(ch.nodes.size());
    for (int ci : kids) lf.W[ci].assign((size_t)ch.nodes[ci].A2.in * P, 0.0);
    for (int c = 0; c < pn.in_dim; ++c) {
        const int pc = pa.conn[pn.in_off + c], ci = owner[pc], k = pc - col0[ci];
        const Aff& A2 = ch.nodes[ci].A2;
        const double* w1 = &pn.A1.W[(size_t)c * P];
        const double d = A2.b[k] - pn.A1.a[c];
        for (int o = 0; o < P; ++o) lf.bias[o] += d * w1[o];
        std::vector<double>& W = lf.W[ci];
        for (int e = 0; e < A2.in; ++e) {
            const double w2 = A2.W[(size_t)e * A2.out + k];
            if (w2 == 0.0) continue;
            for (int o = 0; o < P; ++o) W[(size_t)e * P + o] += w2 * w1[o];
        }
    }
    for (int ci : kids) {
        const Aff& A2 = ch.nodes[ci].A2;
        for (int e = 0; e < A2.in; ++e) {
            const double a = A2.a[e];
            if (a == 0.0) continue;
            for (int o = 0; o < P; ++o) lf.bias[o] -= a * lf.W[ci][(size_t)e * P + o];
        }
    }
    return lf;
}

}

std::vector<int> hoist_first_affines(std::vector<FStage>& fs, const FusedOptions& opt) {
    (void)opt;
    std::vector<int> parents;
    auto ordinary = [](const FStage& st) {
        for (auto& n : st.nodes)
            if (n.is_ig || n.has_prod || n.has_clip || !n.has_exp) return false;
        return true;
    };
    auto rem_tile = [](int d) {
        const int r = d - 16 * ((d + 15) / 16 - 1);
        return r >= 1 && r <= 4;
    };
    for (size_t l = 1; l + 1 < fs.size(); ++l) {
        FStage& ch = fs[l];
        FStage& pa = fs[l + 1];
        if (!ordinary(ch) || !ordinary(pa)) continue;
        const int nc = (int)ch.nodes.size(), np = (int)pa.nodes.size();
        std::vector<int> owner, col0(nc, 0);
        for (int ci = 0; ci < nc; ++ci) {
            col0[ci] = (int)owner.size();
            owner.insert(owner.end(), ch.nodes[ci].out_dim, ci);
        }
        std::vector<int> reads(owner.size(), 0), parent_of(nc, -1);
        std::vector<std::vector<int>> kids(np);
        bool ok = true;
        int p_max = 0;
        for (int pj = 0; pj < np && ok; ++pj) {
            const FNode& pn = pa.nodes[pj];
            p_max = std::max(p_max, pn.A1.out);
            if (pn.A1.in != pn.in_dim || !pn.sum_bias.empty()) ok = false;
            for (int c = 0; c < pn.in_dim && ok; ++c) {
                const int pc = pa.conn[pn.in_off + c];
                if (pc < 0 || pc >= (int)owner.size() || ++reads[pc] > 1) { ok = false; break; }
                const int ci = owner[pc];
                if (parent_of[ci] < 0) {
                    parent_of[ci] = pj;
                    kids[pj].push_back(ci);
                } else if (parent_of[ci] != pj) {
                    ok = false;
                }
            }
            if (kids[pj].empty() || kids[pj].size() > 8) ok = false;
        }
        for (int r : reads) ok = ok && r == 1;
        for (int ci = 0; ci < nc && ok; ++ci) {
            if (parent_of[ci] < 0) { ok = false; break; }
            const FNode& cn = ch.nodes[ci];
            if (cn.A2.out != cn.out_dim || pa.nodes[parent_of[ci]].A1.out > cn.A2.out) ok = false;
        }
        if (!ok || rem_tile(p_max)) continue;

        for (int pj = 0; pj < np; ++pj) {
            FNode& pn = pa.nodes[pj];
            const int P = pn.A1.out;
            LinkFold lf = fold_link(ch, pa, pj, owner, col0, kids[pj]);
            pn.sum_bias = std::move(lf.bias);
            pn.kids = kids[pj];
            std::vector<std::vector<double>>& Wf = lf.W;
            for (int ci : kids[pj]) {
                FNode& cn = ch.nodes[ci];
                Aff f;
                f.in = cn.A2.in;
                f.out = P;
                f.a.assign(f.in, 0.0);
                f.W = std::move(Wf[ci]);
                f.b.assign(P, 0.0);
                cn.A2 = std::move(f);
                cn.out_dim = P;
            }
            pn.A1.a.clear();
            pn.A1.W.clear();
            pn.A1.b.clear();
        }
        ch.out_w = 0;
        for (auto& cn : ch.nodes) ch.out_w += cn.out_dim;
        pa.sum_in = true;
        parents.push_back((int)l + 1);
    }
    return parents;
}

namespace {

inline int q_of_row(int i) { return 4 * (i & 3) + (i >> 2); }

constexpr int kStage0ChunkCols = 128;
struct Planner : FusedPlan {
    Planner(const TNode& root, std::vector<FStage>&& fs, const FusedOptions& options) {
        opt = options;
        out_dim = root.out_dim;
        std::vector<int32_t> prev_blk, prev_q;
        int prev_nb = 0;
        bool prev_packed = false;
        for (size_t si = 0; si < fs.size(); ++si) {
            FStage& st = fs[si];
            if (st.nodes[0].is_ig) {
                if (stages.empty()) add_gather0(st, prev_blk, prev_q, prev_nb);
                build_ig_stage(st, prev_blk, prev_q, prev_nb);
                prev_packed = false;
                continue;
            }
            {
                bool table_driven = st.nodes[0].has_clip;
                for (auto& nd : st.nodes) table_driven = table_driven || nd.has_prod;
                if (table_driven) {
                    if (stages.empty()) add_gather0(st, prev_blk, prev_q, prev_nb);
                    build_prod_stage(st, prev_blk, prev_q, prev_nb, (int)si);
                    prev_packed = false;
                    continue;
                }
            }
            if (si > 0 && stages.empty()) fail(HG_ERR_FORMAT, "internal: stage order");
            stages.emplace_back();
            HostStage& hs = stages.back();
            hs.from_x = si == 0;
            const int n = (int)st.nodes.size();
            hs.n_nodes = n;
            hs.has_exp = st.nodes[0].has_exp;
            hs.funcs = st.nodes[0].funcs;
            hs.nf = (int)hs.funcs.size();
            int p_max = 0;
            for (auto& nd : st.nodes) {
                hs.mt1 = std::max(hs.mt1, (nd.A1.out + 15) / 16);
                if (nd.has_exp) hs.mt2 = std::max(hs.mt2, (nd.A2.out + 15) / 16);
                p_max = std::max(p_max, nd.A1.out);
                if (nd.has_exp) hs.s_max = std::max(hs.s_max, nd.A2.out);
            }
            hs.p_max = p_max;
            if (!hs.has_exp) hs.mt2 = 1;
            hs.mto = hs.has_exp ? hs.mt2 : hs.mt1;
            hs.nb_in = prev_nb;
            for (int mt1 = 0; mt1 < hs.mt1; ++mt1)
                for (int fi = 0; fi < hs.nf; ++fi) {
                    int valid = std::max(0, std::min(16, hs.funcs[fi].used(p_max) - 16 * mt1));
                    hs.nk2[mt1][fi] = (uint8_t)((valid + 3) / 4);
                }

            struct NodeK {
                std::vector<int> src, nk;
                std::vector<std::vector<int>> kpos;
            };
            std::vector<NodeK> nks(n);
            if (si == 0) plan_stage0_inputs(st, hs);
            for (int ni = 0; ni < n; ++ni) {
                FNode& nd = st.nodes[ni];
                NodeK& K = nks[ni];
                if (st.sum_in) {
                    const HostStage& below = stages[stages.size() - 2];
                    if (below.kind != 0 || below.pack_out || below.mto != hs.mt1) fail(HG_ERR_FORMAT, "internal: hoisted link over a layer of another layout");
                    for (int ci : nd.kids)
                        for (int mt = 0; mt < hs.mt1; ++mt) {
                            K.src.push_back(ci * below.mto + mt);
                            K.nk.push_back(1);
                            for (int qq = 0; qq < 16; ++qq) K.kpos.emplace_back();
                        }
                } else if (si == 0) {
                    const int nkb = (nd.in_dim + 15) / 16;
                    for (int kb = 0; kb < nkb; ++kb) {
                        int valid = std::min(16, nd.in_dim - kb * 16), nk = 0;
                        K.src.push_back(0);
                        for (int q = 0; q < 16; ++q) {
                            K.kpos.emplace_back();
                            const int pos = s0_pos(q >> 2, q & 3);
                            if (pos < valid) {
                                K.kpos.back().push_back(kb * 16 + pos);
                                nk = std::max(nk, (q >> 2) + 1);
                            }
                        }
                        K.nk.push_back(nk);
                    }
                } else {
                    std::map<int, int> blk_index;
                    for (int c = 0; c < nd.in_dim; ++c) {
                        int pc = st.conn[nd.in_off + c];
                        int blk = prev_blk[pc], q = prev_q[pc];
                        auto it = blk_index.find(blk);
                        int kb;
                        if (it == blk_index.end()) {
                            kb = (int)K.src.size();
                            blk_index[blk] = kb;
                            K.src.push_back(blk);
                            K.nk.push_back(0);
                            for (int qq = 0; qq < 16; ++qq) K.kpos.emplace_back();
                        } else {
                            kb = it->second;
                        }
                        K.kpos[kb * 16 + q].push_back(c);
                        K.nk[kb] = std::max(K.nk[kb], q / 4 + 1);
                    }
                }
                hs.kb1 = std::max(hs.kb1, (int)K.src.size());
            }
            hs.sum_in = st.sum_in;
            hs.n_kids = st.sum_in ? hs.kb1 / hs.mt1 : 0;
            const int a1_blocks = st.sum_in ? 0 : hs.kb1 * hs.mt1;
            hs.node_blocks = a1_blocks + (hs.has_exp ? hs.mt1 * hs.nf * hs.mt2 : 0);
            hs.bias_floats = (hs.mt1 + (hs.has_exp ? hs.mt2 : 0)) * 16;
            if (si > 0 && (size_t)hs.node_blocks * 1024 + (size_t)hs.bias_floats * 4 + (size_t)hs.kb1 * 8 > 150 * 1024)
                fail(HG_ERR_FORMAT, "fused: one node needs %d KiB of weight fragments, more than a workgroup's LDS", hs.node_blocks);
            hs.afrag.assign((size_t)n * hs.node_blocks * 256, 0.f);
            hs.bias.assign((size_t)n * hs.bias_floats, 0.f);
            if (si > 0) hs.kb1tab.assign((size_t)n * hs.kb1 * 2, 0);

            std::vector<int32_t> cur_blk, cur_q, node_out;
            for (int ni = 0; ni < n; ++ni) {
                FNode& nd = st.nodes[ni];
                NodeK& K = nks[ni];
                const int p = nd.A1.out;
                float* wnode = hs.afrag.data() + (size_t)ni * hs.node_blocks * 256;
                float* bnode = hs.bias.data() + (size_t)ni * hs.bias_floats;
                std::vector<double> bias1 = st.sum_in ? nd.sum_bias : nd.A1.b;
                for (int c = 0; c < nd.in_dim && !st.sum_in; ++c) {
                    double av = si == 0 ? nd.A1.a[c] - (double)(float)nd.A1.a[c] : nd.A1.a[c];
                    if (av == 0.0) continue;
                    for (int o = 0; o < p; ++o) bias1[o] -= av * nd.A1.W[(size_t)c * p + o];
                }
                for (size_t kb = 0; kb < K.src.size(); ++kb) {
                    int r0 = 0;
                    if (si > 0 && prev_packed) {
                        r0 = 4;
                        for (int q = 0; q < 16; ++q)
                            if (!K.kpos[kb * 16 + q].empty()) r0 = std::min(r0, q / 4);
                        if (r0 >= K.nk[kb]) r0 = 0;
                    }
                    if (si > 0) {
                        hs.kb1tab[((size_t)ni * hs.kb1 + kb) * 2] = K.src[kb];
                        hs.kb1tab[((size_t)ni * hs.kb1 + kb) * 2 + 1] = K.nk[kb] | (r0 << 8);
                    }
                    if (st.sum_in) continue;
                    hs.mfma_per_tile += (int64_t)(K.nk[kb] - r0) * hs.mt1;
                    hs.ks1_tile += K.nk[kb] - r0;
                    for (int mt = 0; mt < hs.mt1; ++mt) {
                        float* blk = wnode + ((size_t)kb * hs.mt1 + mt) * 256;
                        for (int lane = 0; lane < 64; ++lane) {
                            int i = lane & 15, gg = lane >> 4;
                            int fo = 16 * mt + q_of_row(i);
                            if (fo >= p) continue;
                            for (int r = 0; r < 4; ++r) {
                                double w = 0;
                                for (int c : K.kpos[kb * 16 + 4 * r + gg]) w += nd.A1.W[(size_t)c * p + fo];
                                blk[lane * 4 + r] = (float)w;
                            }
                        }
                    }
                }
                if (si > 0)
                    for (int kb = (int)K.src.size(); kb < hs.kb1; ++kb) hs.kb1tab[((size_t)ni * hs.kb1 + kb) * 2] = K.src[0];
                if (si == 0 && (int)K.src.size() == hs.kb1) hs.nk_last = std::max(ni == 0 ? 0 : hs.nk_last, K.nk.back());
                for (int mt = 0; mt < hs.mt1; ++mt)
                    for (int gg = 0; gg < 4; ++gg)
                        for (int r = 0; r < 4; ++r) {
                            int fo = 16 * mt + 4 * r + gg;
                            bnode[mt * 16 + gg * 4 + r] = fo < p ? (float)bias1[fo] : 0.f;
                        }
                int n_out = p;
                if (hs.has_exp) {
                    const int s = nd.A2.out;
                    n_out = s;
                    std::vector<int> foff(nd.funcs.size());
                    int eo = 0;
                    for (size_t fi = 0; fi < nd.funcs.size(); ++fi) {
                        foff[fi] = eo;
                        eo += nd.funcs[fi].out_dim(p);
                    }
                    if (eo != nd.A2.in) fail(HG_ERR_DIM, "fused: expansion width %d != second affine input_dim %d", eo, nd.A2.in);
                    std::vector<double> bias2 = nd.A2.b;
                    for (int c = 0; c < nd.A2.in; ++c)
                        for (int o = 0; o < s; ++o) bias2[o] -= nd.A2.a[c] * nd.A2.W[(size_t)c * s + o];
                    float* w2 = wnode + (size_t)a1_blocks * 256;
                    for (int mt1 = 0; mt1 < hs.mt1; ++mt1)
                        for (int fi = 0; fi < hs.nf; ++fi) {
                            const int used = nd.funcs[fi].used(p);
                            hs.mfma_per_tile += (int64_t)hs.nk2[mt1][fi] * hs.mt2;
                            hs.ks2_tile += hs.nk2[mt1][fi];
                            for (int mt2 = 0; mt2 < hs.mt2; ++mt2) {
                                float* blk = w2 + ((size_t)(mt1 * hs.nf + fi) * hs.mt2 + mt2) * 256;
                                for (int lane = 0; lane < 64; ++lane) {
                                    int i = lane & 15, gg = lane >> 4;
                                    int fo = 16 * mt2 + q_of_row(i);
                                    if (fo >= s) continue;
                                    for (int r = 0; r < 4; ++r) {
                                        int fz = 16 * mt1 + 4 * r + gg;
                                        if (fz >= used) continue;
                                        blk[lane * 4 + r] = (float)nd.A2.W[(size_t)(foff[fi] + fz) * s + fo];
                                    }
                                }
                            }
                        }
                    for (int mt = 0; mt < hs.mt2; ++mt)
                        for (int gg = 0; gg < 4; ++gg)
                            for (int r = 0; r < 4; ++r) {
                                int fo = 16 * mt + 4 * r + gg;
                                bnode[hs.mt1 * 16 + mt * 16 + gg * 4 + r] = fo < s ? (float)bias2[fo] : 0.f;
                            }
                }
                node_out.push_back(n_out);
            }
            {
                const int r1 = hs.p_max - 16 * (hs.mt1 - 1), r2 = hs.s_max - 16 * (hs.mt2 - 1);
                hs.rem4 = si >= 1 && hs.has_exp && n > 4 && hs.mt1 == hs.mt2 && (hs.mt1 == 2 || hs.mt1 == 3) && r1 >= 1 && r1 <= 4 &&
                          r2 >= 1 && r2 <= 4 && !opt.no_rem4 && !st.sum_in;
                if (hs.rem4) {
                    auto to4x4 = [](float* blk) {
                        float old[256];
                        std::copy(blk, blk + 256, old);
                        for (int l = 0; l < 64; ++l) {
                            const int src = (l & 48) | ((l & 3) << 2);
                            for (int r = 0; r < 4; ++r) blk[l * 4 + r] = old[src * 4 + r];
                        }
                    };
                    for (int ni = 0; ni < n; ++ni) {
                        float* wnode = hs.afrag.data() + (size_t)ni * hs.node_blocks * 256;
                        for (int kb = 0; kb < hs.kb1; ++kb) to4x4(wnode + ((size_t)kb * hs.mt1 + hs.mt1 - 1) * 256);
                        float* w2 = wnode + (size_t)hs.kb1 * hs.mt1 * 256;
                        for (int b2 = 0; b2 < hs.mt1 * hs.nf; ++b2) to4x4(w2 + ((size_t)b2 * hs.mt2 + hs.mt2 - 1) * 256);
                    }
                }
            }
            hs.pack_out = false;
            if (hs.rem4 && n % 4 == 0 && !opt.no_pack && si + 1 < fs.size()) {
                const FStage& nx = fs[si + 1];
                bool ok = nx.nodes.size() > 16;
                for (auto& nd : nx.nodes) ok = ok && !nd.is_ig && !nd.has_prod && !nd.has_clip && nd.has_exp;
                hs.pack_out = ok;
            }
            if (hs.pack_out) {
                const FStage& nx = fs[si + 1];
                std::vector<int> col0(n, 0), reader(n, 1 << 30);
                for (int ni = 1; ni < n; ++ni) col0[ni] = col0[ni - 1] + node_out[ni - 1];
                std::vector<int> owner;
                for (int ni = 0; ni < n; ++ni) owner.insert(owner.end(), node_out[ni], ni);
                for (size_t pj = 0; pj < nx.nodes.size(); ++pj)
                    for (int c = 0; c < nx.nodes[pj].in_dim; ++c) {
                        const int col = nx.conn[nx.nodes[pj].in_off + c];
                        const int ni = owner[col];
                        if (col - col0[ni] >= 16 * (hs.mto - 1)) reader[ni] = std::min(reader[ni], (int)pj);
                    }
                std::vector<int> order(n);
                for (int ni = 0; ni < n; ++ni) order[ni] = ni;
                std::stable_sort(order.begin(), order.end(), [&](int a, int b) { return reader[a] < reader[b]; });
                hs.pack_slot.assign(n, 0);
                for (int rk = 0; rk < n; ++rk) hs.pack_slot[order[rk]] = rk;
            }
            for (int ni = 0; ni < n; ++ni)
                for (int f = 0; f < node_out[ni]; ++f) {
                    if (hs.pack_out && f >= 16 * (hs.mto - 1)) {
                        cur_blk.push_back(n * (hs.mto - 1) + hs.pack_slot[ni] / 4);
                        cur_q.push_back(4 * (hs.pack_slot[ni] % 4) + (f - 16 * (hs.mto - 1)));
                    } else {
                        cur_blk.push_back(ni * (hs.pack_out ? hs.mto - 1 : hs.mto) + f / 16);
                        cur_q.push_back(f % 16);
                    }
                }
            hs.nb_out = hs.pack_out ? n * (hs.mto - 1) + n / 4 : n * hs.mto;
            prev_packed = hs.pack_out;
            prev_blk.swap(cur_blk);
            prev_q.swap(cur_q);
            prev_nb = hs.nb_out;
            max_nb = std::max(max_nb, hs.nb_out);
            {
                const bool front_rem = si == 1 && hs.has_exp && hs.mt1 == 2 && hs.mt2 == 2 && hs.p_max <= 20 && hs.s_max <= 20 && hs.nk2[1][0] <= 1 &&
                                       hs.nk2[1][1] <= 1 && !opt.no_rem4;
                const int rem = (hs.rem4 || front_rem) ? 1 : 0;
                hs.mfma16_tile = hs.ks1_tile * (hs.mt1 - rem) + (hs.has_exp ? hs.ks2_tile * (hs.mt2 - rem) : 0);
                hs.mfma4_tile = rem ? hs.ks1_tile + hs.ks2_tile : 0;
            }
            padded_flops += (hs.mfma16_tile * 2048 + hs.mfma4_tile * 512) / 16;
            std::ostringstream os;
            os << "fused stage " << si << (hs.rem4 ? (hs.pack_out ? " (4x4 remainder tiles, packed four to a block)" : " (4x4 remainder tiles)") : "") << ": " << hs.n_nodes << " nodes, K-blocks " << hs.kb1 << ", tiles " << hs.mt1 << "x" << hs.mt2
               << (hs.sum_in ? " (first affine folded into the layer below's second, plain 16-row tiles only: z = bias + the tiles of " + std::to_string(hs.n_kids) + " children)" : "")
               << ", " << hs.mfma_per_tile << " MFMA/tile (issued: " << hs.mfma16_tile << " x 16x16x4 + " << hs.mfma4_tile << " x 4x4x1), " << hs.afrag.size() * 4 / 1024
               << " KiB weights, out " << hs.nb_out << " blocks/tile";
            hs.name = os.str();
            if (st.sum_in && opt.pair) plan_pairs(st, hs);
        }
        plan_slot_major();
        fuse01 = can_fuse01();
        if (fuse01) {
            stages[0].name += "  [+ stage 1 fused in the same persistent kernel when the input allows 16-byte loads]";
        }
        if (opt.fold01) plan_fold01(fs);
        if (opt.fold01_pack) plan_fold01_pack(fs);
        col_base.resize(out_dim);
        col_of.assign((size_t)std::max(prev_nb, 1) * 16, -1);
        for (int c = 0; c < out_dim; ++c) {
            int q = prev_q[c];
            col_base[c] = prev_blk[c] * 256 + (q & 3) * 64 + (q >> 2);
            col_of[(size_t)prev_blk[c] * 16 + q] = c;
        }
        for (auto& hs : stages)
            if (!hs.kb1tab.empty()) hs.kb1tab.resize(hs.kb1tab.size() + 16, 0);
        plan_tail();
        plan_subtree();
        for (auto& hs : stages)
            if (!hs.chunks.empty()) hs.piece_col.resize(std::max<size_t>(hs.piece_col.size(), 2));
    }

    void plan_pairs(const FStage& st, HostStage& hs) {
        size_t lo = ~(size_t)0, hi = 0;
        for (auto& nd : st.nodes) {
            lo = std::min(lo, nd.kids.size());
            hi = std::max(hi, nd.kids.size());
        }
        if (lo != 2 || hi != 2) {
            hs.name += lo == hi ? "; unpaired: " + std::to_string(lo) + " children per node" : "; unpaired: " + std::to_string(lo) + " to " + std::to_string(hi) + " children per node";
            return;
        }
        const int n = hs.n_nodes;
        hs.pair_kids.reserve((size_t)n * 2);
        for (auto& nd : st.nodes) {
            hs.pair_kids.push_back(nd.kids[0]);
            hs.pair_kids.push_back(nd.kids[1]);
        }
        hs.kb1tab_pre.assign(((size_t)n * hs.mt1 + 8) * 2, 0);
        for (int ni = 0; ni < n; ++ni)
            for (int mt = 0; mt < hs.mt1; ++mt) {
                hs.kb1tab_pre[((size_t)ni * hs.mt1 + mt) * 2] = ni * hs.mt1 + mt;
                hs.kb1tab_pre[((size_t)ni * hs.mt1 + mt) * 2 + 1] = 1;
            }
        hs.bias_pre = hs.bias;
        for (int ni = 0; ni < n; ++ni) std::fill_n(hs.bias_pre.begin() + (size_t)ni * hs.bias_floats, hs.mt1 * 16, -0.0f);
        hs.name += "; paired: the layer below may store (bias + child 0) + child 1 once per node where both layers run the node-group sweep";
    }

    void plan_stage0_inputs(const FStage& st, HostStage& hs) {
        const int n = (int)st.nodes.size();
        int kb1 = 0, max_in = 0;
        for (auto& nd : st.nodes) {
            kb1 = std::max(kb1, (nd.in_dim + 15) / 16);
            max_in = std::max(max_in, nd.in_dim);
        }
        s0_transpose = true;
        for (auto& nd : st.nodes) {
            for (int c = 0; c < nd.in_dim && s0_transpose; c += 4)
                for (int r = 1; r < 4 && c + r < nd.in_dim; ++r)
                    if (st.conn[nd.in_off + c + r] != st.conn[nd.in_off + c] + r) s0_transpose = false;
            if (nd.in_dim % 4) s0_transpose = false;
        }
        const int col_budget = std::max(kStage0ChunkCols, (max_in + 3) / 4 * 4);
        if (col_budget > 2048) fail(HG_ERR_FORMAT, "fused: first-layer node with %d inputs", max_in);
        hs.koff.assign((size_t)n * kb1 * 16, -1);
        hs.kmean.assign((size_t)n * kb1 * 16, 0.f);
        int max_cols = 0, ni = 0;
        bool vec_ok = true, contig = true;
        while (ni < n) {
            std::vector<int32_t> cols;
            int n1 = ni;
            while (n1 < n) {
                std::vector<int32_t> c2 = cols;
                const FNode& nd = st.nodes[n1];
                for (int c = 0; c < nd.in_dim; ++c) c2.push_back(st.conn[nd.in_off + c]);
                std::sort(c2.begin(), c2.end());
                c2.erase(std::unique(c2.begin(), c2.end()), c2.end());
                if ((int)c2.size() > col_budget && n1 > ni) break;
                cols.swap(c2);
                ++n1;
            }
            DChunk ck{ni, n1 - ni, (int)hs.runs.size(), 0, 0, (int)hs.piece_col.size() / 2, 0, 0};
            std::map<int32_t, int32_t> lds_of;
            int n_runs = 0, max_len = 0;
            for (size_t i = 0; i < cols.size();) {
                size_t k = i + 1;
                while (k < cols.size() && cols[k] == cols[k - 1] + 1) ++k;
                ++n_runs;
                max_len = std::max(max_len, (int)(k - i));
                i = k;
            }
            const bool packed4 = s0_transpose && n_runs == 4 && max_len <= 32;
            static const int packed_off[4] = {0, 64, 32, 96};
            int off = 0, run_i = 0, hi = 0;
            for (size_t i = 0; i < cols.size(); ++run_i) {
                size_t k = i + 1;
                while (k < cols.size() && cols[k] == cols[k - 1] + 1) ++k;
                const int len = (int)(k - i);
                off = packed4 ? packed_off[run_i] : (off + 63) / 64 * 64;
                hs.runs.push_back(DRun{cols[i], len, off, 0});
                if (cols[i] % 4 || len % 4) vec_ok = false;
                for (size_t m = i; m < k; ++m) lds_of[cols[m]] = off + (int)(m - i);
                for (int pc = 0; pc + 3 < len; pc += 4) {
                    hs.piece_col.push_back(cols[i] + pc);
                    hs.piece_col.push_back(off + pc);
                    ++ck.n_pieces;
                }
                off += len;
                hi = std::max(hi, off);
                i = k;
                ++ck.run_count;
            }
            off = hi;
            ck.n_cols = off;
            max_cols = std::max(max_cols, off);
            for (int k = ni; k < n1; ++k) {
                const FNode& nd = st.nodes[k];
                for (int kb = 0; kb < kb1; ++kb)
                    for (int g = 0; g < 4; ++g)
                        for (int r = 0; r < 4; ++r) {
                            int c = kb * 16 + s0_pos(r, g);
                            size_t e = (((size_t)k * kb1 + kb) * 4 + g) * 4 + r;
                            if (c < nd.in_dim) {
                                hs.koff[e] = lds_of[st.conn[nd.in_off + c]];
                                hs.kmean[e] = (float)nd.A1.a[c];
                            }
                        }
            }
            hs.chunks.push_back(ck);
            hs.max_chunk_nodes = std::max(hs.max_chunk_nodes, ck.node_count);
            hs.max_chunk_pieces = std::max(hs.max_chunk_pieces, ck.n_pieces);
            ni = n1;
        }
        int stride = max_cols + 1;
        while (stride % 64 != 4) ++stride;
        hs.lds_stride = stride;
        for (size_t e = 0; e < hs.koff.size(); e += 4) {
            bool any_pad = false;
            for (int r = 0; r < 4; ++r)
                if (hs.koff[e + r] < 0) {
                    hs.koff[e + r] = stride - 1;
                    any_pad = true;
                }
            if (any_pad || hs.koff[e] % 4) contig = false;
            for (int r = 1; r < 4; ++r)
                if (hs.koff[e + r] != hs.koff[e] + r) contig = false;
        }
        hs.contig4 = contig;
        hs.vec_ok = vec_ok;
        bool direct = contig && vec_ok && s0_transpose && kb1 == 1;
        hs.kcol.assign((size_t)n * 4, 0);
// ... 281 lines not shown
        }
        struct NodeK {
            std::vector<int> src, nk;
            std::vector<std::vector<int>> kpos;
        };
        std::vector<NodeK> nks(n);
        for (int ni = 0; ni < n; ++ni) {
            FNode& nd = st.nodes[ni];
            NodeK& K = nks[ni];
            std::map<int, int> blk_index;
            for (int c = 0; c < nd.in_dim; ++c) {
                const int pc = st.conn[nd.in_off + c], blk = prev_blk[pc], q = prev_q[pc];
                auto it = blk_index.find(blk);
                int kb;
                if (it == blk_index.end()) {
                    kb = (int)K.src.size();
                    blk_index[blk] = kb;
                    K.src.push_back(blk);
                    K.nk.push_back(0);
                    for (int qq = 0; qq < 16; ++qq) K.kpos.emplace_back();
                } else {
                    kb = it->second;
                }
                K.kpos[kb * 16 + q].push_back(c);
                K.nk[kb] = std::max(K.nk[kb], q / 4 + 1);
            }
            hs.kb1 = std::max(hs.kb1, (int)K.src.size());
        }
        hs.node_blocks = hs.kb1 * hs.mt1 + (hs.mt1 * hs.nf + hs.neb) * hs.mt2;
        hs.bias_floats = (hs.mt1 + hs.mt2) * 16;
        if ((size_t)hs.node_blocks * 1024 + (size_t)hs.bias_floats * 4 + (size_t)hs.kb1 * 8 + (size_t)hs.neb * 128 + (size_t)4 * hs.mt1 * 1024 > 150 * 1024)
            fail(HG_ERR_FORMAT, "fused: one node needs %d KiB of weight fragments (%d product columns), more than a workgroup's LDS", hs.node_blocks, E);
        hs.afrag.assign((size_t)n * hs.node_blocks * 256, 0.f);
        hs.bias.assign((size_t)n * hs.bias_floats, 0.f);
        hs.kb1tab.assign((size_t)n * hs.kb1 * 2, 0);
        std::vector<int32_t> cur_blk, cur_q;
        for (int ni = 0; ni < n; ++ni) {
            FNode& nd = st.nodes[ni];
            NodeK& K = nks[ni];
            const int p = nd.A1.out, sdim = nd.A2.out;
            float* wnode = hs.afrag.data() + (size_t)ni * hs.node_blocks * 256;
            float* bnode = hs.bias.data() + (size_t)ni * hs.bias_floats;
            std::vector<double> bias1 = nd.A1.b;
            for (int c = 0; c < nd.in_dim; ++c)
                for (int o = 0; o < p; ++o) bias1[o] -= nd.A1.a[c] * nd.A1.W[(size_t)c * p + o];
            for (int kb = 0; kb < hs.kb1; ++kb) {
                const bool real = kb < (int)K.src.size();
                hs.kb1tab[((size_t)ni * hs.kb1 + kb) * 2] = real ? K.src[kb] : K.src[0];
                hs.kb1tab[((size_t)ni * hs.kb1 + kb) * 2 + 1] = real ? K.nk[kb] : 0;
                if (!real) continue;
                hs.mfma_per_tile += (int64_t)K.nk[kb] * hs.mt1;
                for (int mt = 0; mt < hs.mt1; ++mt) {
                    float* blk = wnode + ((size_t)kb * hs.mt1 + mt) * 256;
                    for (int lane = 0; lane < 64; ++lane) {
                        const int i = lane & 15, gg = lane >> 4, fo = 16 * mt + q_of_row(i);
                        if (fo >= p) continue;
                        for (int r = 0; r < 4; ++r) {
                            double w = 0;
                            for (int c : K.kpos[kb * 16 + 4 * r + gg]) w += nd.A1.W[(size_t)c * p + fo];
                            blk[lane * 4 + r] = (float)w;
                        }
                    }
                }
            }
            for (int mt = 0; mt < hs.mt1; ++mt)
                for (int gg = 0; gg < 4; ++gg)
                    for (int r = 0; r < 4; ++r) {
                        const int fo = 16 * mt + 4 * r + gg;
                        bnode[mt * 16 + gg * 4 + r] = fo < p ? (float)bias1[fo] : 0.f;
                    }
            std::vector<int> foff(nf_all);
            int eo = 0;
            for (int fi = 0; fi < nf_all; ++fi) {
                foff[fi] = eo;
                eo += all[fi].out_dim(p);
            }
            if (eo != nd.A2.in) fail(HG_ERR_DIM, "fused: expansion width %d != second affine input_dim %d", eo, nd.A2.in);
            std::map<std::tuple<int, int, int>, int> row_of;
            {
                const std::vector<Col> cn = products(p);
                std::vector<int> cnt(nf_all, 0);
                for (auto& c : cn) row_of[std::make_tuple(c.fi, c.i, c.k)] = foff[c.fi] + cnt[c.fi]++;
            }
            std::vector<double> bias2 = nd.A2.b;
            for (int c = 0; c < nd.A2.in; ++c)
                for (int o = 0; o < sdim; ++o) bias2[o] -= nd.A2.a[c] * nd.A2.W[(size_t)c * sdim + o];
            float* w2 = wnode + (size_t)hs.kb1 * hs.mt1 * 256;
            for (int mt1 = 0; mt1 < hs.mt1; ++mt1)
                for (int fa = 0; fa < nf_all; ++fa) {
                    const int fi = elem_of[fa];
                    if (fi < 0) continue;
                    const int used = all[fa].used(p);
                    hs.mfma_per_tile += (int64_t)hs.nk2[mt1][fi] * hs.mt2;
                    for (int mt2 = 0; mt2 < hs.mt2; ++mt2) {
                        float* blk = w2 + ((size_t)(mt1 * hs.nf + fi) * hs.mt2 + mt2) * 256;
                        for (int lane = 0; lane < 64; ++lane) {
                            const int i = lane & 15, gg = lane >> 4, fo = 16 * mt2 + q_of_row(i);
                            if (fo >= sdim) continue;
                            for (int r = 0; r < 4; ++r) {
                                const int fz = 16 * mt1 + 4 * r + gg;
                                if (fz >= used) continue;
                                blk[lane * 4 + r] = (float)nd.A2.W[(size_t)(foff[fa] + fz) * sdim + fo];
                            }
                        }
                    }
                }
            float* wp = w2 + (size_t)hs.mt1 * hs.nf * hs.mt2 * 256;
            for (int eb = 0; eb < hs.neb; ++eb) {
                hs.mfma_per_tile += (int64_t)(eb + 1 < hs.neb ? 4 : hs.nk_last) * hs.mt2;
                for (int mt2 = 0; mt2 < hs.mt2; ++mt2) {
                    float* blk = wp + ((size_t)eb * hs.mt2 + mt2) * 256;
                    for (int lane = 0; lane < 64; ++lane) {
                        const int i = lane & 15, gg = lane >> 4, fo = 16 * mt2 + q_of_row(i);
                        if (fo >= sdim) continue;
                        for (int r = 0; r < 4; ++r) {
                            const int c = 16 * eb + 4 * r + gg;
                            if (c >= E) continue;
                            auto it = row_of.find(std::make_tuple(cmax[c].fi, cmax[c].i, cmax[c].k));
                            if (it == row_of.end()) continue;
                            blk[lane * 4 + r] = (float)nd.A2.W[(size_t)it->second * sdim + fo];
                        }
                    }
                }
            }
            for (int mt = 0; mt < hs.mt2; ++mt)
                for (int gg = 0; gg < 4; ++gg)
                    for (int r = 0; r < 4; ++r) {
                        const int fo = 16 * mt + 4 * r + gg;
                        bnode[hs.mt1 * 16 + mt * 16 + gg * 4 + r] = fo < sdim ? (float)bias2[fo] : 0.f;
                    }
            for (int f = 0; f < sdim; ++f) {
                cur_blk.push_back(ni * hs.mto + f / 16);
                cur_q.push_back(f % 16);
            }
        }
        hs.nb_out = n * hs.mto;
        prev_blk.swap(cur_blk);
        prev_q.swap(cur_q);
        prev_nb = hs.nb_out;
        max_nb = std::max(max_nb, hs.nb_out);
        padded_flops += hs.mfma_per_tile * 2048 / 16;
        std::ostringstream os;
        os << "fused stage " << si << " (table-driven expansion: products" << (hs.has_clip ? ", clip" : "") << "): " << n << " nodes, K-blocks " << hs.kb1
           << ", tiles " << hs.mt1 << "x" << hs.mt2 << ", " << hs.nf << " element-wise functions, " << E << " product columns in " << hs.neb
           << " K-blocks, " << hs.mfma_per_tile << " MFMA/tile, " << hs.afrag.size() * 4 / 1024 << " KiB weights";
        hs.name = os.str();
    }

    void plan_slot_major() {
        if (opt.no_soa) return;
        for (size_t si = 0; si + 1 < stages.size(); ++si) {
            HostStage& pr = stages[si];
            HostStage& co = stages[si + 1];
            if (!pr.pack_out || co.kind != 0 || !co.rem4 || co.kb1 != 3 || co.mt1 != co.mt2 || (co.mt1 != 2 && co.mt1 != 3)) continue;
            const int base = pr.n_nodes * (pr.mto - 1);
            int pk = -1;
            bool ok = true;
            for (int ni = 0; ni < co.n_nodes && ok; ++ni) {
                int seen = 0;
                for (int kb = 0; kb < co.kb1; ++kb) {
                    const int src = co.kb1tab[((size_t)ni * co.kb1 + kb) * 2], y = co.kb1tab[((size_t)ni * co.kb1 + kb) * 2 + 1];
                    if (src < base) continue;
                    const int nk = y & 255, r0 = y >> 8;
                    ++seen;
                    if (nk == 0 || nk - r0 > 2 || (pk >= 0 && pk != kb)) ok = false;
                    pk = kb;
                }
                if (seen != 1) ok = false;
            }
            if (!ok || pk != 1) continue;
            for (int ni = 0; ni < co.n_nodes; ++ni) {
                int32_t& y = co.kb1tab[((size_t)ni * co.kb1 + pk) * 2 + 1];
                const int nk = y & 255, r0 = y >> 8;
                float* wnode = co.afrag.data() + (size_t)ni * co.node_blocks * 256;
                for (int mt = 0; mt < co.mt1; ++mt) {
                    float* blk = wnode + ((size_t)pk * co.mt1 + mt) * 256;
                    for (int lane = 0; lane < 64; ++lane) {
                        float v[4] = {0.f, 0.f, 0.f, 0.f};
                        for (int r = r0; r < nk; ++r) v[r - r0] = blk[lane * 4 + r];
                        for (int r = 0; r < 4; ++r) blk[lane * 4 + r] = v[r];
                    }
                }
                y = (nk - r0) | (r0 << 16);
            }
            pr.pack_soa = true;
            co.pack_in = base;
            co.pk_kbi = pk;
            pr.name += "  [packed blocks slot-major]";
        }
    }

    void plan_tail() {
        tail_begin = -1;
        if (opt.tail_max <= 0) return;
        const int ns = (int)stages.size();
        int b = ns;
        int act_blocks = 0, e_blocks = 0;
        while (b > (fuse01 ? 2 : 1) && ns - b < opt.tail_max) {
            const HostStage& s = stages[b - 1];
            if (s.kind != 0 || s.from_x || s.rem4 || s.pack_out || s.pk_kbi >= 0 || s.pack_in != INT32_MAX || s.nf > kMaxFuncs) break;
            if (s.has_exp && s.mt1 * s.nf > 8) break;
            const int waves = s.n_nodes * (s.has_exp ? std::max(s.mt1, s.mt2) : s.mt1);
            if (waves > 16) break;
            const int act = b - 1 < ns - 1 ? std::max(act_blocks, s.nb_out) : act_blocks;
            const int eb = std::max(e_blocks, s.has_exp ? s.n_nodes * s.nf * s.mt1 : 0);
            if (((size_t)2 * act + eb) * 1024 > 150 * 1024) break;
            act_blocks = act;
            e_blocks = eb;
            --b;
        }
        if (b == ns) return;
        tail_begin = b;
        tail_act_blocks = act_blocks;
        tail_e_blocks = e_blocks;
        for (int i = b; i < ns; ++i)
            stages[i].name += i == b ? (ns - b > 1 ? "  [this and the layers above: ONE launch, activations in LDS, writes the caller's rows]"
                                                    : "  [writes the caller's rows: no unpack pass]")
                                      : "  [in the top-of-hierarchy launch]";
    }

    void plan_subtree() {
        sub_runs.clear();
        if (opt.subtree_max_tiles <= 0) return;
        const int ns = (int)stages.size();
        const int end = tail_begin < 0 ? ns : (ns - tail_begin >= 3 ? tail_begin + 1 : tail_begin);
        plan_subtree_set(end, 0);
        if (!sub_runs.empty()) plan_subtree_set(end - 1, 1);
    }

    void plan_subtree_set(int end, int set) {
        while (end - 1 >= 2) {
            const int last = end - 1;
            const int k = stages[last].n_nodes;
            int b = last + 1, act_blocks = 0, e_blocks = 0;
            std::vector<std::vector<int32_t>> members(kMaxTail), tabs(kMaxTail);
            while (k >= 4 && b > (fuse01 ? 2 : 1) && last + 1 - b < kMaxTail) {
                const HostStage& s = stages[b - 1];
                if (s.kind != 0 || s.from_x || s.rem4 || s.pack_out || s.pk_kbi >= 0 || s.pack_in != INT32_MAX || s.nf > kMaxFuncs ||
                    s.n_nodes % k)
                    break;
                if (s.has_exp && s.mt1 * s.nf > 8) break;
                const int per = s.n_nodes / k;
                if (per * (s.has_exp ? std::max(s.mt1, s.mt2) : s.mt1) > 16) break;
                std::vector<int32_t> mem((size_t)k * per, -1), tab;
                if (b - 1 == last) {
                    for (int j = 0; j < k; ++j) mem[j] = j;
                } else {
                    const HostStage& up = stages[b];
                    const std::vector<int32_t>& mup = members[last - b];
                    const int per_up = up.n_nodes / k;
                    std::vector<int32_t> owner(s.n_nodes, -1), pos(s.n_nodes, -1);
                    bool ok = s.nb_out == s.n_nodes * s.mto;
                    tab.assign(up.kb1tab.size(), 0);
                    for (int j = 0; j < k && ok; ++j) {
                        int have = 0;
                        for (int q = 0; q < per_up && ok; ++q) {
                            const int ni = mup[(size_t)j * per_up + q];
                            for (int kb = 0; kb < up.kb1 && ok; ++kb) {
                                const size_t at = ((size_t)ni * up.kb1 + kb) * 2;
                                const int src = up.kb1tab[at];
                                if (src < 0 || src >= s.nb_out) { ok = false; break; }
                                const int sn = src / s.mto;
                                if (owner[sn] < 0) {
                                    if (have == per) { ok = false; break; }
                                    owner[sn] = j;
                                    pos[sn] = have;
                                    mem[(size_t)j * per + have++] = sn;
                                } else if (owner[sn] != j) {
                                    ok = false;
                                    break;
                                }
                                tab[at] = pos[sn] * s.mto + src % s.mto;
                                tab[at + 1] = up.kb1tab[at + 1];
                            }
                        }
                        if (have != per) ok = false;
                    }
                    if (!ok) break;
                }
                const int act = b - 1 < last ? std::max(act_blocks, per * s.mto) : act_blocks;
                const int eb = std::max(e_blocks, s.has_exp ? per * s.nf * s.mt1 : 0);
                if (((size_t)2 * act + eb) * 1024 > 150 * 1024) break;
                act_blocks = act;
                e_blocks = eb;
                members[last - (b - 1)] = std::move(mem);
                if (b - 1 < last) tabs[last - b] = std::move(tab);
                --b;
            }
            if (last + 1 - b < 2) {
                end = last;
                continue;
            }
            SubRun r;
            r.begin = b;
            r.len = last + 1 - b;
            r.n = k;
            r.act_blocks = act_blocks;
            r.e_blocks = e_blocks;
            r.set = set;
            for (int i = b; i <= last; ++i) {
                r.nodes[i - b] = members[last - i];
                if (i > b) r.tab[i - b] = tabs[last - i];
            }
            sub_runs.push_back(std::move(r));
            if (set != 0) {
                stages[b].name += "  [or, where more layers or more sub-trees can run that way: " + std::to_string(last + 1 - b) + " layers from here as " + std::to_string(k) + " sub-trees]";
                end = b;
                continue;
            }
            for (int i = b; i <= last; ++i) {
                stages[i].name += i == b ? "  [batches of up to " + std::to_string(std::min(opt.subtree_max_tiles, opt.subtree_max_wgs / k) * 16) + " rows: this and the next " +
                                                std::to_string(last - b) + " layer(s) as " + std::to_string(k) + " sub-trees in ONE launch]"
                                          : "  [in the sub-tree launch for short batches]";
            }
            end = b;
        }
    }

    void plan_fold01(const std::vector<FStage>& fs) {
        if (stages.size() < 2) return;
        auto refuse = [&](const std::string& why) {
            fold01_note = "link 0 -> 1 stays as it is: " + why;
            stages[1].name += "  [" + fold01_note + "]";
        };
        if (!fuse01) {
            bool ig = false;
            for (size_t l = 0; l < 2 && l < fs.size(); ++l)
                for (auto& n : fs[l].nodes) ig = ig || n.is_ig || n.was_ig;
            return refuse(ig ? "an iGSFA front end" : "layers 0 and 1 do not share the front kernel");
        }
        const FStage &ch = fs[0], &pa = fs[1];
        HostStage &a = stages[0], &b = stages[1];
        for (auto& n : pa.nodes)
            if (n.was_ig) return refuse("layer 1 is an iGSFA layer (identity first affine, no remainder tiles)");
        for (auto& n : ch.nodes)
            if (n.was_ig) return refuse("layer 0 is an iGSFA layer");
        auto id_pow = [](const HostStage& hs) { return hs.nf == 2 && hs.funcs[0].kind == E_IDENTITY && hs.funcs[1].kind == E_ABS_POW; };
        if (!id_pow(a) || !id_pow(b)) return refuse("both layers must expand with exactly (identity, |x|^p)");
        if (opt.no_rem4) return refuse("4x4 remainder tiles are switched off (HIGSFA_NO_REM4)");
        if (!(b.p_max >= 17 && b.p_max <= 20 && b.s_max >= 17 && b.s_max <= 20 && b.nk2[1][0] <= 1 && b.nk2[1][1] <= 1))
            return refuse("layer 1 has no 4x4 remainder tiles (affines of " + std::to_string(b.p_max) + " and " + std::to_string(b.s_max) + " outputs, not 17..20)");
        const int nc = (int)ch.nodes.size(), np = (int)pa.nodes.size();
        std::vector<int> owner, col0(nc, 0);
        for (int ci = 0; ci < nc; ++ci) {
            col0[ci] = (int)owner.size();
            owner.insert(owner.end(), ch.nodes[ci].out_dim, ci);
        }
        for (int q = 0; q < np; ++q) {
            const FNode& pn = pa.nodes[q];
            if (pn.A1.in != pn.in_dim) return refuse("internal: layer-1 first affine");
            for (int c = 0; c < pn.in_dim; ++c) {
                const int pc = pa.conn[pn.in_off + c];
                if (pc < 0 || pc >= (int)owner.size() || owner[pc] >> 1 != q) return refuse("a layer-1 node reads other nodes than 2n and 2n + 1");
            }
        }
        b.fold_frag.assign((size_t)np * 8 * 256, 0.f);
        b.fold_bias.assign((size_t)np * 32, 0.f);
        auto to4x4 = [](float* blk) {
            float old[256];
            std::copy(blk, blk + 256, old);
            for (int l = 0; l < 64; ++l) {
                const int src = (l & 48) | ((l & 3) << 2);
                for (int r = 0; r < 4; ++r) blk[l * 4 + r] = old[src * 4 + r];
            }
        };
        for (int q = 0; q < np; ++q) {
            const FNode& pn = pa.nodes[q];
            const int P = pn.A1.out;
            const LinkFold lf = fold_link(ch, pa, q, owner, col0, {2 * q, 2 * q + 1});
            for (int sl = 0; sl < 2; ++sl) {
                const FNode& cn = ch.nodes[2 * q + sl];
                const std::vector<double>& F = lf.W[2 * q + sl];
                const int p0 = cn.A1.out;
                int eo = 0;
                for (int fi = 0; fi < 2; ++fi) {
                    const int used = cn.funcs[fi].used(p0);
                    for (int mt = 0; mt < 2; ++mt) {
                        float* blk = b.fold_frag.data() + ((((size_t)q * 2 + sl) * 2 + fi) * 2 + mt) * 256;
                        for (int lane = 0; lane < 64; ++lane) {
                            const int i = lane & 15, gg = lane >> 4;
                            const int fo = 16 * mt + q_of_row(i);
                            if (fo >= P) continue;
                            for (int r = 0; r < 4; ++r) {
                                const int fz = 4 * r + gg;
                                if (fz >= used) continue;
                                blk[lane * 4 + r] = (float)F[(size_t)(eo + fz) * P + fo];
                            }
                        }
                        if (mt == 1) to4x4(blk);
                    }
                    eo += cn.funcs[fi].out_dim(p0);
// ... 22 lines not shown
        b.name += "  [" + fold01_note + "]";
    }

    void plan_fold01_pack(const std::vector<FStage>& fs) {
        if (stages.size() < 2) return;
        auto refuse = [&](const std::string& why) {
            fold01_pack_note = "the link's one-row k-steps stay as they are: " + why;
            stages[1].name += "  [" + fold01_pack_note + "]";
        };
        if (!fold01) return refuse(opt.fold01 ? "the link 0 -> 1 stays as it is" : "the link 0 -> 1 stays as it is (fold01 is off)");
        const FStage& ch = fs[0];
        HostStage &a = stages[0], &b = stages[1];
        for (auto& n : ch.nodes) {
            const int p0 = n.A1.out;
            if (p0 != 13)
                return refuse("a layer-0 node has " + std::to_string(p0) + " outputs, not 13 (4 m + 1: one feature alone in the last register)");
            if (n.funcs[0].used(p0) != p0 || n.funcs[1].used(p0) != p0) return refuse("a layer-0 function does not expand all 13 outputs");
        }
        if (a.kb1 != 1 || a.mt1 != 1 || a.bias_floats < 16) return refuse("internal: layer 0's first affine is not one block");
        const int nc = a.n_nodes, np = b.n_nodes;
        a.fold_a1.assign((size_t)nc * 256, 0.f);
        a.fold_b1.assign((size_t)nc * 16, 0.f);
        for (int ci = 0; ci < nc; ++ci) {
            const float* blk = a.afrag.data() + (size_t)ci * a.node_blocks * 256;
            const float* bias = a.bias.data() + (size_t)ci * a.bias_floats;
            float* nb = a.fold_a1.data() + (size_t)ci * 256;
            float* bb = a.fold_b1.data() + (size_t)ci * 16;
            std::copy_n(blk, 256, nb);
            std::copy_n(bias, 16, bb);
            for (int row : {7, 11, 15}) {
                bool zero = bias[row] == 0.f;
                for (int g = 0; g < 4; ++g)
                    for (int r = 0; r < 4; ++r) zero = zero && blk[((g * 16 + row) * 4) + r] == 0.f;
                if (!zero) fail(HG_ERR_FORMAT, "internal: a padding row of layer 0's first affine is in use");
            }
            auto copy_row = [&](int to) {
                for (int g = 0; g < 4; ++g)
                    for (int r = 0; r < 4; ++r) nb[((g * 16 + to) * 4) + r] = blk[((g * 16 + 3) * 4) + r];
                bb[to] = bias[3];
            };
            if (ci & 1) {
                copy_row(7);
                copy_row(15);
                for (int g = 0; g < 4; ++g)
                    for (int r = 0; r < 4; ++r) nb[((g * 16 + 3) * 4) + r] = 0.f;
                bb[3] = 0.f;
            } else {
                copy_row(11);
            }
        }
        b.fold_last.assign((size_t)np * 2 * 64, 0.f);
        for (int q = 0; q < np; ++q)
            for (int sl = 0; sl < 2; ++sl)
                for (int fi = 0; fi < 2; ++fi)
                    for (int mt = 0; mt < 2; ++mt) {
                        float* blk = b.fold_frag.data() + ((((size_t)q * 2 + sl) * 2 + fi) * 2 + mt) * 256;
                        const int g = 2 * fi + sl;
                        for (int i = 0; i < 16; ++i) b.fold_last[((size_t)q * 2 + mt) * 64 + g * 16 + i] = blk[i * 4 + 3];
                        for (int lane = 0; lane < 64; ++lane) blk[lane * 4 + 3] = 0.f;
                    }
        const int64_t before = padded_flops;
        b.mfma16_tile -= 3 * (int64_t)np;
        b.mfma4_tile -= 3 * (int64_t)np;
        padded_flops -= (3 * (int64_t)np * 2048 + 3 * (int64_t)np * 512) / 16;
        fold01_flops += padded_flops - before;
        fold01_pack = true;
        fold01_pack_note = "one-row k-steps packed: feature 12 of both children and both functions in ONE k-step behind twelve full ones, this layer then issues " +
                           std::to_string(b.mfma16_tile) + " x 16x16x4 + " + std::to_string(b.mfma4_tile) + " x 4x4x1";
        b.name += "  [" + fold01_pack_note + "]";
    }

    bool can_fuse01() const {
        if (stages.size() < 2) return false;
        const HostStage& a = stages[0];
        const HostStage& b = stages[1];
        if (a.kind != 0 || b.kind != 0 || !a.from_x) return false;
        if (!(a.has_exp && a.mt1 == 1 && a.mt2 == 1 && a.kb1 == 1 && a.nf == 2 && a.contig4 && a.vec_ok)) return false;
        if (a.nk_last != 4 || a.nk2[0][0] != 4 || a.nk2[0][1] != 4) return false;
        if (a.max_chunk_nodes > 16 || a.max_chunk_pieces > 64) return false;
        for (auto& c : a.chunks)
            if ((c.node_begin & 1) || (c.node_count & 1)) return false;
        if (!(b.has_exp && b.mt1 == 2 && b.mt2 == 2 && b.kb1 == 2 && b.nf == 2 && b.nk2[0][0] == 4 && b.nk2[0][1] == 4)) return false;
        if (b.n_nodes * 2 != a.n_nodes) return false;
        for (int n = 0; n < b.n_nodes; ++n)
            if (b.kb1tab[(size_t)n * 4] != 2 * n || b.kb1tab[(size_t)n * 4 + 2] != 2 * n + 1) return false;
        return true;
    }

    int s0_pos(int r, int g) const { return s0_transpose ? 4 * g + r : 4 * r + g; }
};

}

bool FusedPlan::sub_run_pays(const SubRun& r, int n_tiles) const {
    return n_tiles <= opt.subtree_max_tiles && (int64_t)r.n * n_tiles <= opt.subtree_max_wgs;
}

int FusedPlan::pick_sub_set(int n_tiles) const {
    int best = 0, best_cov = -1, best_k = 0;
    for (int set = 0; set < 2; ++set) {
        int cov = 0, mink = 0x7fffffff;
        for (const SubRun& r : sub_runs)
            if (r.set == set && sub_run_pays(r, n_tiles)) {
                cov += r.len;
                mink = std::min(mink, r.n);
            }
        if (cov > best_cov || (cov == best_cov && cov > 0 && mink > best_k)) {
            best = set;
            best_cov = cov;
            best_k = mink;
        }
    }
    return best;
}

int FusedPlan::tail_start(int n_tiles) const {
    const int ns = (int)stages.size();
    bool short_batch = n_tiles < 96;
    const int sub_set = pick_sub_set(n_tiles);
    for (const SubRun& r : sub_runs)
        if (r.set == sub_set && r.begin <= tail_begin && tail_begin < r.begin + r.len && sub_run_pays(r, n_tiles)) short_batch = true;
    return (ns - tail_begin >= 3 && short_batch) ? tail_begin + 1 : tail_begin;
}

std::unique_ptr<const FusedPlan> build_fused_plan(const TNode& root, const FusedOptions& opt, std::string* why_not) {
    std::vector<FStage> stages;
    std::string why;
    if (!build_stages(root, stages, why, opt)) {
        if (why_not) *why_not = why;
        return nullptr;
    }
    for (auto& st : stages) {
        const FNode& f0 = st.nodes[0];
        bool table_driven = f0.has_clip;
        for (auto& n : st.nodes) table_driven = table_driven || n.has_prod;
        if (f0.funcs.size() > (size_t)kMaxFuncs && !table_driven) {
            if (why_not) *why_not = "more than 4 expansion functions";
            return nullptr;
        }
        for (auto& n : st.nodes) {
            bool same = n.has_exp == f0.has_exp && n.is_ig == f0.is_ig && n.funcs.size() == f0.funcs.size() && n.has_clip == f0.has_clip &&
                        (!n.has_clip || (n.clip_lo == f0.clip_lo && n.clip_hi == f0.clip_hi));
            for (size_t i = 0; same && i < n.funcs.size(); ++i)
                same = n.funcs[i].kind == f0.funcs[i].kind && n.funcs[i].expo == f0.funcs[i].expo && n.funcs[i].sel == f0.funcs[i].sel &&
                       n.funcs[i].k == f0.funcs[i].k;
            if (!same) {
                if (why_not) *why_not = "nodes of one layer use different expansions";
                return nullptr;
            }
        }
    }
    if (why_not) why_not->clear();
    int64_t given = -1;
    if (opt.hoist) {
        std::vector<FStage> plain = stages;
        if (!hoist_first_affines(stages, opt).empty()) {
            try {
                FusedOptions o = opt;
                o.hoist = false;
                o.fold01 = false;
                o.fold01_pack = false;
                given = Planner(root, std::move(plain), o).padded_flops;
            } catch (const Error&) {
            }
        }
    }
    try {
        Planner p(root, std::move(stages), opt);
        p.padded_flops_given = given >= 0 ? given : p.padded_flops - p.fold01_flops;
        return std::make_unique<const FusedPlan>(std::move(static_cast<FusedPlan&>(p)));
    } catch (const Error& e) {
        if (why_not) *why_not = e.what();
        return nullptr;
    }
}

}
}
```

### pyfaceanalysis_amd/csrc/hg_fused_plan.hpp

```cpp
#pragma once
#include <algorithm>
#include <cstdlib>

#include "hg_common.hpp"

namespace hg {
namespace fused {

constexpr int kMaxMT = 4;

constexpr int kMaxFuncs = 4;

constexpr int kMaxTail = 3;

struct DChunk {
    int32_t node_begin, node_count, run_begin, run_count, n_cols, piece_begin, n_pieces, pad1;
};
struct DRun {
    int32_t start, len, lds_off, pad;
};

struct FusedOptions {
    bool no_rem4 = false, ig_nofold = false, debug = false;
    int stamp_stage = -1;
    bool no_pack = false;
    bool no_soa = false;
    uint32_t wq_start = 0;
    bool no_wgq = false;
    bool no_direct = false;
    int tail_max = 3;
    bool no_fspec = false;
    int subtree_max_tiles = 64;
    int subtree_max_wgs = 256;
    int splitm_max_nodes = 4;
    int splitm_max_wgs = 512;
    int sum_lds_kib = 32;
    bool hoist = false;
    bool fold01 = false;
    bool fold01_pack = false;
    bool pair = false;
    int pair_min_wgs = 512;
    static FusedOptions from_env() {
        FusedOptions o;
        o.no_rem4 = getenv("HIGSFA_NO_REM4") != nullptr;
        o.ig_nofold = getenv("HIGSFA_IG_NOFOLD") != nullptr;
        o.debug = getenv("HIGSFA_DEBUG") != nullptr;
        if (const char* e = getenv("HIGSFA_STAMP")) o.stamp_stage = atoi(e);

        o.no_pack = getenv("HIGSFA_NO_PACK") != nullptr;
        o.no_soa = getenv("HIGSFA_NO_SOA") != nullptr;
        o.no_fspec = getenv("HIGSFA_NO_FSPEC") != nullptr;
        o.no_direct = getenv("HIGSFA_NO_DIRECT") != nullptr;
        o.no_wgq = getenv("HIGSFA_NO_WGQ") != nullptr;
        if (const char* e = getenv("HIGSFA_WQ_START")) o.wq_start = (uint32_t)strtoul(e, nullptr, 0);
        if (const char* e = getenv("HIGSFA_SPLITM_MAX")) o.splitm_max_nodes = atoi(e);
        if (const char* e = getenv("HIGSFA_SPLITM_WGS")) o.splitm_max_wgs = atoi(e);
        if (const char* e = getenv("HIGSFA_SUBTREE")) o.subtree_max_tiles = std::max(0, atoi(e));
        if (const char* e = getenv("HIGSFA_SUBTREE_WGS")) o.subtree_max_wgs = std::max(0, atoi(e));
        if (const char* e = getenv("HIGSFA_SUM_LDS")) o.sum_lds_kib = std::max(1, atoi(e));
        if (const char* e = getenv("HIGSFA_PAIR_WGS")) o.pair_min_wgs = std::max(0, atoi(e));
        if (const char* e = getenv("HIGSFA_TAIL")) o.tail_max = std::max(0, std::min(atoi(e), kMaxTail));
        return o;
    }
};

struct SubRun {
    int begin = 0, len = 0, n = 0, act_blocks = 0, e_blocks = 0, set = 0;
    std::vector<int32_t> nodes[kMaxTail], tab[kMaxTail];
};

struct HostStage {
    int mt1 = 1, mt2 = 1, mto = 1, nb_out = 0, nb_in = 0, n_nodes = 0, kb1 = 0, nf = 0;
    int node_blocks = 0, bias_floats = 0, nk_last = 4;
    int p_max = 0, s_max = 0;
    bool rem4 = false;
    bool pack_out = false;
    bool pack_soa = false;
    int pack_in = 0x7fffffff;
    int pk_kbi = -1;
    std::vector<int32_t> pack_slot;
    bool has_exp = false, contig4 = false, vec_ok = false;
    std::vector<ExpFunc> funcs;
    uint8_t nk2[kMaxMT][kMaxFuncs] = {};
    std::vector<float> afrag, bias;
    std::vector<int32_t> kb1tab;
    std::vector<DChunk> chunks;
    std::vector<DRun> runs;
    std::vector<int32_t> piece_col, koff;
    std::vector<float> kmean;
    std::vector<int32_t> kcol;
    bool direct_ok = false;
    int lds_stride = 0, max_chunk_nodes = 0, max_chunk_pieces = 0;
    int kind = 0;
    int neb = 0;
    bool has_clip = false;
    float clip_lo = 0, clip_hi = 0;
    std::vector<int32_t> etab;
    bool from_x = false;
    bool ig_has_lr = false, ig_folded = false;
    int ig_nks[kMaxMT] = {};
    std::vector<int32_t> gcol;
    int64_t mfma_per_tile = 0;
    int64_t mfma16_tile = 0, mfma4_tile = 0;
    int64_t ks1_tile = 0, ks2_tile = 0;
    std::string name;
    bool sum_in = false;
    int n_kids = 0;
    std::vector<float> fold_frag, fold_bias;
    std::vector<float> fold_last, fold_a1, fold_b1;
    std::vector<int32_t> pair_kids;
    std::vector<int32_t> kb1tab_pre;
    std::vector<float> bias_pre;
};

struct FusedPlan {
    FusedOptions opt;
    int out_dim = 0;
    bool s0_transpose = false, fuse01 = false;
    bool fold01 = false;
    std::string fold01_note;
    bool fold01_pack = false;
    std::string fold01_pack_note;
    std::vector<HostStage> stages;
    std::vector<int32_t> col_base, col_of;
    int tail_begin = -1;
    int tail_act_blocks = 0, tail_e_blocks = 0;
    std::vector<SubRun> sub_runs;
    int max_nb = 0;
    int64_t padded_flops = 0;
    int64_t fold01_flops = 0;
    int64_t padded_flops_given = 0;

    bool sub_run_pays(const SubRun& r, int n_tiles) const;
    int pick_sub_set(int n_tiles) const;
    int tail_start(int n_tiles) const;
};

std::unique_ptr<const FusedPlan> build_fused_plan(const TNode& root, const FusedOptions& opt, std::string* why_not);

}
}
```

### pyfaceanalysis_amd/csrc/hg_fused_stages.hpp

```cpp
#pragma once
#include <string>
#include <vector>

#include "hg_fused_plan.hpp"

namespace hg {
namespace fused {

struct Aff {
    int in = 0, out = 0;
    std::vector<double> a, W, b;
};

struct FNode {
    int in_off = 0, in_dim = 0, out_dim = 0;
    Aff A1, A2;
    bool has_exp = false;
    std::vector<ExpFunc> funcs;
    bool has_prod = false;
    bool has_clip = false;
    double clip_lo = 0, clip_hi = 0;
    bool is_ig = false, ig_has_lr = false;
    bool was_ig = false;
    int ig_k = 0;
    std::vector<double> ig_mean;
    Aff ig_sfa, ig_lr, ig_pca;
    std::vector<int> kids;
    std::vector<double> sum_bias;
};

struct FStage {
    std::vector<int32_t> conn;
    std::vector<FNode> nodes;
    int out_w = 0;
    bool sum_in = false;
};

bool build_stages(const TNode& root, std::vector<FStage>& stages, std::string& why, const FusedOptions& opt);

std::vector<int> hoist_first_affines(std::vector<FStage>& stages, const FusedOptions& opt);

}
}
```

Baseline: 10.18 million sub-images/s.

## Add pair-folded stage sweep computing both children and parent first affine once

Adds a new FoldPair route and kernel. For each parent node, one pass over both children computes their first affine and expansion, then accumulates directly into the parent's first-affine tile set through the folded second affine. Each parent's z is stored once, so the child outputs are never written or re-read, and the parent stage reads a single precomputed tile set. The cost is a specialised kernel (3x4 tiles, 3 K-blocks, packed block 1, T=2 only), more LDS per group, and added planner complexity, including a fail path when the shape does not match.

```diff
diff --git a/pyfaceanalysis_amd/build.py b/pyfaceanalysis_amd/build.py
--- a/pyfaceanalysis_amd/build.py
+++ b/pyfaceanalysis_amd/build.py
@@ -7,7 +7,7 @@
 HERE = os.path.dirname(os.path.abspath(__file__))
 CSRC = os.path.join(HERE, "csrc")
 LIB = os.path.join(HERE, "libhigsfa.so")
-SOURCES = ["hg_tree.cpp", "hg_capi.cpp", "hg_hostpack.cpp", "hg_resample.cpp", "hg_normalize.cpp", "hg_normalize.hip", "hg_generic.hip", "hg_fused_plan.cpp", "hg_fused_call.cpp", "hg_fused.hip", "hg_fused_sum.hip", "hg_fused_front.hip", "hg_fused_igsfa.hip", "hg_fused_prod.hip", "hg_fused_tail.hip",
+SOURCES = ["hg_tree.cpp", "hg_capi.cpp", "hg_hostpack.cpp", "hg_resample.cpp", "hg_normalize.cpp", "hg_normalize.hip", "hg_generic.hip", "hg_fused_plan.cpp", "hg_fused_call.cpp", "hg_fused.hip", "hg_fused_sum.hip", "hg_fused_foldpair.hip", "hg_fused_front.hip", "hg_fused_igsfa.hip", "hg_fused_prod.hip", "hg_fused_tail.hip",
            "hg_gauss.hip", "hg_extract.hip", "hg_resample.hip", "hg_cascade.hip", "hg_eyes.hip", "hg_estimate.hip", "hg_train.hip"]
 HEADERS = ["hg_common.hpp", os.path.join("..", "..", "include", "higsfa.h")]
 HOST_ONLY = {"hg_hostpack.cpp": [], "hg_resample.cpp": ["-ffp-contract=off"], "hg_normalize.cpp": ["-ffp-contract=off"]}
diff --git a/pyfaceanalysis_amd/csrc/hg_fused.hip b/pyfaceanalysis_amd/csrc/hg_fused.hip
--- a/pyfaceanalysis_amd/csrc/hg_fused.hip
+++ b/pyfaceanalysis_amd/csrc/hg_fused.hip
@@ -550,6 +550,7 @@
     DevBuf fold_frag, fold_bias;
     DevBuf fold_last;
     DevBuf pair_kids, kb1tab_pre, bias_pre;
+    DevBuf fold_pairs, fold_pair_bias;
 };
 struct SubRunDev {
     DevBuf nodes[kMaxTail], tab[kMaxTail];
@@ -636,6 +637,10 @@
                 d.pair_kids.upload(s.pair_kids.data(), s.pair_kids.size() * 4);
                 d.kb1tab_pre.upload(s.kb1tab_pre.data(), s.kb1tab_pre.size() * 4);
                 d.bias_pre.upload(s.bias_pre.data(), s.bias_pre.size() * 4);
+            }
+            if (!s.fold_pairs.empty()) {
+                d.fold_pairs.upload(s.fold_pairs.data(), s.fold_pairs.size() * 4);
+                d.fold_pair_bias.upload(s.fold_pair_bias.data(), s.fold_pair_bias.size() * 4);
             }
             if (!s.chunks.empty()) {
                 d.chunks.upload(s.chunks.data(), s.chunks.size() * sizeof(DChunk));
@@ -744,6 +749,7 @@
                 case Route::Front0: launch_front(step, s, d, P, x, x_dtype, ldx, n, st); break;
                 case Route::ProdSweep: launch_prod(step, s, d, P, st); break;
                 case Route::Splitm: launch_splitm(step, s, P, st); break;
+                case Route::FoldPair: launch_stage_fold_pair(step, s, d, P, st); break;
                 default:
                     if (step.in_summed) {
                         P.kb1tab = (const int2*)d.kb1tab_pre.p;
@@ -1061,6 +1067,19 @@
         hipLaunchKernelGGL(fn, (unsigned)blocks, sh.threads, sh.lds, st, P);
     }
 
+    void launch_stage_fold_pair(const CallStep& step, const HostStage& s, const StageDev& d, StageParams& P, hipStream_t st) {
+        const CallShape& sh = step.sh;
+        StageFn fn = s.rem1 && s.pack_in != INT32_MAX ? pick_stage_fold_pair(s.mt1, s.mt2, s.kb1, s.pk_kbi, sh.T) : nullptr;
+        if (!fn || !d.fold_pairs.p || !d.fold_pair_bias.p)
+            fail(HG_ERR_STATE, "fused: no pair sweep for a pair-folded stage of %d x %d tiles, %d K-blocks, packed block at %d, %d tiles per wave", s.mt1, s.mt2, s.kb1, s.pk_kbi, sh.T);
+        P.pair_kids = (const int2*)d.fold_pairs.p;
+        P.pair_bias = (const float*)d.fold_pair_bias.p;
+        P.pair_bias_floats = s.mto * 16;
+        P.n_pairs = (int)s.fold_pairs.size() / 2;
+        const int64_t blocks = fill_sweep(step, fn, P);
+        hipLaunchKernelGGL(fn, (unsigned)blocks, sh.threads, sh.lds, st, P);
+    }
+
     void launch_prod(const CallStep& step, const HostStage& s, const StageDev& d, StageParams& P, hipStream_t st) {
         StageFn fn = pick_prod(s.mt1, s.mt2, step.sh.T);
         const int64_t blocks = fill_sweep(step, fn, P);
diff --git a/pyfaceanalysis_amd/csrc/hg_fused_call.cpp b/pyfaceanalysis_amd/csrc/hg_fused_call.cpp
--- a/pyfaceanalysis_amd/csrc/hg_fused_call.cpp
+++ b/pyfaceanalysis_amd/csrc/hg_fused_call.cpp
@@ -14,6 +14,7 @@
     opt.fold01 = getenv("HIGSFA_NO_FOLD01") == nullptr;
     opt.fold01_pack = opt.fold01 && getenv("HIGSFA_NO_FOLD01_PACK") == nullptr;
     opt.pair = opt.hoist && getenv("HIGSFA_NO_PAIR") == nullptr;
+    opt.pair_fold = opt.hoist && getenv("HIGSFA_NO_PAIR_FOLD") == nullptr;
     return opt;
 }
 
@@ -23,7 +24,7 @@
 
 const char* route_name(Route r) {
     static const char* const names[] = {"gather", "front01d", "front01p", "front0p", "front0", "igsweep", "igsplit", "prod", "splitm", "sweep", "sumpair",
-                                        "subtree", "top"};
+                                        "foldpair", "subtree", "top"};
     return names[(int)r];
 }
 
@@ -67,10 +68,12 @@
 }
 bool link_summed(const HostStage& s, const HostStage& p, int n_tiles, bool in_summed, const FusedOptions& opt) {
     if (p.pair_kids.empty() || !s.sum_in || s.n_nodes != 2 * p.n_nodes) return false;
-    if (!in_summed && (s.pair_kids.empty() || s.kb1 != 2 * s.mt1)) return false;
+    const bool one_child = in_summed || (s.fold_parent && s.n_kids == 1 && s.kb1 == s.mt1);
+    if (!one_child && (s.pair_kids.empty() || s.kb1 != 2 * s.mt1)) return false;
     if (!(s.has_exp && fs_expansion(s, opt)) || s.mt1 != 4 || s.mt2 != 4 || p.mt1 != 4 || s.mto != 4 || s.pack_out || s.rem4) return false;
     const int ppg = pair_group(s, opt), nw = pair_waves(n_tiles);
     const int64_t n_groups = (p.n_nodes + ppg - 1) / ppg, tile_groups = (n_tiles + nw * kPairTiles - 1) / (nw * kPairTiles);
+    if (s.fold_parent && tile_groups < opt.pair_min_wgs / 32) return false;
     return n_groups * tile_groups >= opt.pair_min_wgs;
 }
 
@@ -219,6 +222,24 @@
     sh.threads = sh.nw * 64;
     sh.lds = (size_t)2 * ppg * ((size_t)s.node_blocks * 1024 + (size_t)s.bias_floats * 4 + (size_t)sh.kb1 * 8) + (size_t)ppg * 256;
     sh.fs = true;
+}
+
+void shape_fold_pair(const HostStage& s, int n_tiles, CallShape& sh) {
+    const int n_pairs = (int)s.fold_pairs.size() / 2;
+    const size_t per_pair = (size_t)2 * ((size_t)s.node_blocks * 1024 + (size_t)s.bias_floats * 4 + (size_t)s.kb1 * 8) + (size_t)s.mto * 64;
+    int nw = 8;
+    while (nw * kFoldPairTiles > std::max(n_tiles, 1) && nw > 1) nw >>= 1;
+    sh.kb1 = s.kb1;
+    sh.nw = nw;
+    sh.T = kFoldPairTiles;
+    sh.per_group = (int)std::max<size_t>(1, std::min<size_t>(n_pairs, (size_t)72 * 1024 / per_pair));
+    sh.n_groups = ceil_div(n_pairs, sh.per_group);
+    sh.tile_groups = ceil_div(n_tiles, nw * sh.T);
+    sh.threads = nw * 64;
+    sh.lds = (size_t)sh.per_group * per_pair;
+    sh.kbf = s.kb1;
+    sh.fs = true;
+    sh.rem4 = true;
 }
 
 }
@@ -261,6 +282,9 @@
             } else if (s.kind == 3) {
                 st.route = Route::ProdSweep;
                 shape_prod(s, n_tiles, st.sh);
+            } else if (!s.fold_pairs.empty()) {
+                st.route = Route::FoldPair;
+                shape_fold_pair(s, n_tiles, st.sh);
             } else if (splitm_takes(s, n_tiles, plan.opt)) {
                 st.route = Route::Splitm;
                 shape_splitm(s, n_tiles, st.sh);
@@ -307,6 +331,7 @@
     switch (st.route) {
         case Route::Sweep:
         case Route::SumPair:
+        case Route::FoldPair:
         case Route::ProdSweep: return sweep_tile_parts(st.sh.n_groups, st.sh.tile_groups, occ);
         case Route::IgSweep:
         case Route::Front01d:
@@ -320,6 +345,7 @@
     switch (st.route) {
         case Route::Sweep:
         case Route::SumPair:
+        case Route::FoldPair:
         case Route::ProdSweep: {
             const int64_t blocks = (int64_t)((st.sh.n_groups + 7) / 8) * 8 * tile_parts;
             if (blocks > 0x7fffffffll) fail(HG_ERR_ARG, "batch too large");
@@ -378,6 +404,10 @@
             snprintf(buf, cap, "[pair stage %d] pairs %d per group %d shape %dx%d lds %zu tile_groups %d parts %d kids in %d", si, plan.stages[si + 1].n_nodes, sh.per_group,
                      sh.nw, sh.T, sh.lds, sh.tile_groups, tile_parts, sh.n_kids);
             break;
+        case Route::FoldPair:
+            snprintf(buf, cap, "[foldpair stage %d] pairs %d per group %d shape %dx%d lds %zu tile_groups %d parts %d occ %d", si, (int)s.fold_pairs.size() / 2, sh.per_group, sh.nw,
+                     sh.T, sh.lds, sh.tile_groups, tile_parts, occ);
+            break;
         case Route::Subtree: {
             const SubRun& r = plan.sub_runs[st.sub_run];
             snprintf(buf, cap, "[subtree stage %d] layers %d subtrees %d set %d blocks %lld", si, r.len, r.n, r.set, blocks);
diff --git a/pyfaceanalysis_amd/csrc/hg_fused_call.hpp b/pyfaceanalysis_amd/csrc/hg_fused_call.hpp
--- a/pyfaceanalysis_amd/csrc/hg_fused_call.hpp
+++ b/pyfaceanalysis_amd/csrc/hg_fused_call.hpp
@@ -10,6 +10,7 @@
 constexpr int kProdLdsBytes = 52 * 1024;
 constexpr int kPairLdsCapKiB = 144;
 constexpr int kPairTiles = 1;
+constexpr int kFoldPairTiles = 2;
 constexpr bool kDoubleBuffer01 = true;
 constexpr int stage01p_tiles(bool , bool fspec) { return fspec ? 1 : 2; }
 
@@ -29,6 +30,7 @@
     Splitm,
     Sweep,
     SumPair,
+    FoldPair,
     Subtree,
     Top,
 };
diff --git a/pyfaceanalysis_amd/csrc/hg_fused_dev.hpp b/pyfaceanalysis_amd/csrc/hg_fused_dev.hpp
--- a/pyfaceanalysis_amd/csrc/hg_fused_dev.hpp
+++ b/pyfaceanalysis_amd/csrc/hg_fused_dev.hpp
@@ -408,6 +408,7 @@
 StageFn pick_prod(int mt1, int mt2, int T);
 StageFn pick_stage_sum(int mt1, int mt2, int T, bool fs);
 StageFn pick_stage_sum_pair(int T);
+StageFn pick_stage_fold_pair(int mt1, int mt2, int kb1, int pk, int T);
 void launch_igfold_split(const StageParams& P, int mo, int T, unsigned grid, int threads, size_t lds, hipStream_t st);
 void launch_im2frag(const void* x, int x_dtype, int64_t ldx, int64_t n_rows, int n_tiles, int nb, const int32_t* gcol, f32x4* out,
                     int vec4, unsigned grid, hipStream_t st);
diff --git a/pyfaceanalysis_amd/csrc/hg_fused_foldpair.hip b/pyfaceanalysis_amd/csrc/hg_fused_foldpair.hip
--- /dev/null
+++ b/pyfaceanalysis_amd/csrc/hg_fused_foldpair.hip
@@ -0,0 +1,165 @@
+#include <hip/hip_runtime.h>
+
+#include "hg_fused_dev.hpp"
+
+namespace hg {
+namespace fused {
+
+namespace {
+
+template <int T>
+__global__ void __launch_bounds__(512, 4) k_stage_fold_pair(StageParams P) {
+    constexpr int MT1 = 3, MT2 = 4, KBF = 3, PK = 1;
+    extern __shared__ __attribute__((aligned(16))) f32x4 smem[];
+    const int tid = threadIdx.x, nthr = blockDim.x;
+    const int lane = tid & 63, nw = nthr >> 6, g = lane >> 4;
+    const int wave = __builtin_amdgcn_readfirstlane(tid >> 6);
+    const int xcd = blockIdx.x & 7, kq = blockIdx.x >> 3;
+    const int cpx = (P.n_chunks + 7) >> 3;
+    const int chunk = xcd + 8 * (kq % cpx), part = kq / cpx;
+    if (chunk >= P.n_chunks) return;
+    const int ppg = P.nodes_per_group;
+    const int p_begin = chunk * ppg;
+    const int gn = min(ppg, P.n_pairs - p_begin);
+    const int nvn = P.node_blocks * 64, bf = P.bias_floats;
+    float* sb = (float*)(smem + (size_t)2 * ppg * nvn);
+    float* spb = sb + 2 * ppg * bf;
+    int2* stab = (int2*)(spb + ppg * MT2 * 16);
+
+    for (int s = 0; s < 2 * gn; ++s) {
+        const int2 pk = P.pair_kids[p_begin + (s >> 1)];
+        const int node = __builtin_amdgcn_readfirstlane((s & 1) ? pk.y : pk.x);
+        const f32x4* src = P.afrag + (size_t)node * nvn;
+        f32x4* dst = smem + (size_t)s * nvn;
+        int i = tid;
+        for (; i + 7 * nthr < nvn; i += 8 * nthr) {
+            f32x4 v[8];
+#pragma unroll
+            for (int u = 0; u < 8; ++u) v[u] = src[i + u * nthr];
+#pragma unroll
+            for (int u = 0; u < 8; ++u) dst[i + u * nthr] = v[u];
+        }
+        for (; i < nvn; i += nthr) dst[i] = src[i];
+        const float* bsrc = P.bias + (size_t)node * bf;
+        for (int k = tid; k < bf; k += nthr) sb[s * bf + k] = bsrc[k];
+        const int2* tsrc = P.kb1tab + (size_t)node * KBF;
+        for (int k = tid; k < KBF; k += nthr) stab[s * KBF + k] = tsrc[k];
+    }
+    for (int k = tid; k < gn * MT2 * 16; k += nthr) spb[k] = P.pair_bias[(size_t)p_begin * P.pair_bias_floats + k];
+    __syncthreads();
+
+    int tile[T];
+    uint32_t trow[T], trow_nx[T];
+#pragma unroll
+    for (int t = 0; t < T; ++t) tile[t] = (part * nw + wave) * T + t;
+    if (tile[0] >= P.n_tiles) return;
+#pragma unroll
+    for (int t = 0; t < T; ++t) trow[t] = (uint32_t)(tile[t] < P.n_tiles ? tile[t] : tile[0]) * (uint32_t)P.nb_in;
+    f32x4 bq[KBF][T];
+#pragma unroll
+    for (int kbi = 0; kbi < KBF; ++kbi) {
+        const int2 e0 = stab[kbi];
+        const int sb0 = __builtin_amdgcn_readfirstlane(e0.x);
+        if (kbi == PK) load_kblock_soa<T, true>(P, trow, sb0, __builtin_amdgcn_readfirstlane(e0.y), lane, bq[kbi]);
+        else {
+#pragma unroll
+            for (int t = 0; t < T; ++t) bq[kbi][t] = P.in[(size_t)(trow[t] + (uint32_t)sb0) * 64 + lane];
+        }
+    }
+    arrived(bq);
+    const float ex1 = P.expo[1];
+    for (int grp = part; grp < P.tile_groups; grp += P.tile_parts) {
+        const int tn0 = ((grp + P.tile_parts) * nw + wave) * T;
+        const bool has_next = grp + P.tile_parts < P.tile_groups && tn0 < P.n_tiles;
+#pragma unroll
+        for (int t = 0; t < T; ++t) {
+            const int tn = tn0 + t;
+            trow_nx[t] = has_next ? (uint32_t)(tn < P.n_tiles ? tn : tn0) * (uint32_t)P.nb_in : trow[t];
+        }
+        for (int lp = 0; lp < gn; ++lp) {
+            f32x4 y[MT2][T];
+#pragma unroll
+            for (int mt = 0; mt < MT2; ++mt) {
+                const f32x4 bb = *(const f32x4*)(spb + lp * MT2 * 16 + mt * 16 + g * 4);
+#pragma unroll
+                for (int t = 0; t < T; ++t) y[mt][t] = bb;
+            }
+#pragma unroll
+            for (int k = 0; k < 2; ++k) {
+                const int s = 2 * lp + k;
+                const f32x4* wA1 = smem + (size_t)s * nvn + lane;
+                const f32x4* wA2 = wA1 + KBF * MT1 * 64;
+                const float* b1 = sb + s * bf;
+                const int2* kt = stab + s * KBF;
+                f32x4 z[MT1][T];
+#pragma unroll
+                for (int mt = 0; mt < MT1; ++mt) {
+                    const f32x4 bb = *(const f32x4*)(b1 + mt * 16 + g * 4);
+#pragma unroll
+                    for (int t = 0; t < T; ++t) z[mt][t] = bb;
+                }
+                f32x4 d4[T];
+#pragma unroll
+                for (int t = 0; t < T; ++t) d4[t] = f32x4{0.f, 0.f, 0.f, 0.f};
+#pragma unroll
+                for (int kbi = 0; kbi < KBF; ++kbi) {
+                    const int nkr = __builtin_amdgcn_readfirstlane(kt[kbi].y), nk = nkr & 255, r0 = (nkr >> 8) & 255;
+                    gemm_block_rem<MT1, T>(wA1 + kbi * MT1 * 64, bq[kbi], z, d4, nk, r0);
+                }
+#pragma unroll
+                for (int t = 0; t < T; ++t) add_rem4(z[MT1 - 1][t], d4[t]);
+                {
+                    const bool in_group = k == 0 || lp + 1 < gn;
+                    const int2* ktn = in_group ? kt + KBF : stab;
+                    uint32_t rw[T];
+#pragma unroll
+                    for (int t = 0; t < T; ++t) rw[t] = in_group ? trow[t] : trow_nx[t];
+#pragma unroll
+                    for (int kbi = 0; kbi < KBF; ++kbi) {
+                        const int2 en = ktn[kbi];
+                        const int sbn = __builtin_amdgcn_readfirstlane(en.x);
+                        if (kbi == PK) load_kblock_soa<T, true>(P, rw, sbn, __builtin_amdgcn_readfirstlane(en.y), lane, bq[kbi]);
+                        else {
+#pragma unroll
+                            for (int t = 0; t < T; ++t) bq[kbi][t] = P.in[(size_t)(rw[t] + (uint32_t)sbn) * 64 + lane];
+                        }
+                    }
+                }
+#pragma unroll
+                for (int mt1 = 0; mt1 < MT1; ++mt1) {
+                    const uint32_t nkp = P.nk2p[mt1];
+                    const int nk0 = nkp & 15, nk1 = (nkp >> 4) & 15;
+                    gemm_block<MT2, T>(wA2 + (mt1 * 2) * MT2 * 64, z[mt1], y, nk0);
+                    f32x4 e[T];
+#pragma unroll
+                    for (int t = 0; t < T; ++t) e[t] = pow_abs4(z[mt1][t], ex1);
+                    gemm_block<MT2, T>(wA2 + (mt1 * 2 + 1) * MT2 * 64, e, y, nk1);
+                }
+            }
+            const int out_blk = (p_begin + lp) * MT2;
+#pragma unroll
+            for (int mt = 0; mt < MT2; ++mt)
+#pragma unroll
+                for (int t = 0; t < T; ++t) {
+                    const int tl = tile[t] < P.n_tiles ? tile[t] : tile[0];
+                    P.out[((size_t)tl * P.nb_out + out_blk + mt) * 64 + lane] = y[mt][t];
+                }
+        }
+        if (!has_next) break;
+#pragma unroll
+        for (int t = 0; t < T; ++t) {
+            tile[t] = tn0 + t;
+            trow[t] = trow_nx[t];
+        }
+    }
+}
+
+}
+
+StageFn pick_stage_fold_pair(int mt1, int mt2, int kb1, int pk, int T) {
+    if (mt1 == 3 && mt2 == 4 && kb1 == 3 && pk == 1 && T == 2) return (StageFn)k_stage_fold_pair<2>;
+    return nullptr;
+}
+
+}
+}
diff --git a/pyfaceanalysis_amd/csrc/hg_fused_plan.cpp b/pyfaceanalysis_amd/csrc/hg_fused_plan.cpp
--- a/pyfaceanalysis_amd/csrc/hg_fused_plan.cpp
+++ b/pyfaceanalysis_amd/csrc/hg_fused_plan.cpp
@@ -426,6 +426,137 @@
     return parents;
 }
 
+std::vector<int> fold_pair_links(std::vector<FStage>& fs, const std::vector<HostStage>& shapes, const FusedOptions& opt, std::vector<std::string>& notes) {
+    std::vector<int> parents;
+    notes.assign(fs.size(), std::string());
+    if (shapes.size() != fs.size()) return parents;
+    auto ordinary = [](const FStage& st) {
+        for (auto& n : st.nodes)
+            if (n.is_ig || n.has_prod || n.has_clip || !n.has_exp) return false;
+        return true;
+    };
+    auto rem_tile = [](int d) {
+        const int r = d - 16 * ((d + 15) / 16 - 1);
+        return r >= 1 && r <= 4;
+    };
+    for (size_t l = 1; l + 1 < fs.size(); ++l) {
+        FStage& ch = fs[l];
+        FStage& pa = fs[l + 1];
+        if (pa.sum_in) continue;
+        const std::string link = "link " + std::to_string(l) + " -> " + std::to_string(l + 1);
+        std::string& note = notes[l + 1];
+        auto refuse = [&](const std::string& why) { note = link + " stays as it is: " + why; };
+        if (!ordinary(ch) || !ordinary(pa)) {
+            refuse("both layers must be ordinary [affine][element-wise expansion][affine] layers (no product, clip, iGSFA or linear layer)");
+            continue;
+        }
+        if (l < 2) {
+            refuse("the front kernels keep stages 0 and 1 (a stage-1 child's layout is theirs)");
+            continue;
+        }
+        const int nc = (int)ch.nodes.size(), np = (int)pa.nodes.size();
+        std::vector<int> owner, col0(nc, 0);
+        for (int ci = 0; ci < nc; ++ci) {
+            col0[ci] = (int)owner.size();
+            owner.insert(owner.end(), ch.nodes[ci].out_dim, ci);
+        }
+        std::vector<int> reads(owner.size(), 0), parent_of(nc, -1);
+        std::vector<std::vector<int>> kids(np);
+        bool once = true;
+        for (int pj = 0; pj < np && once; ++pj) {
+            const FNode& pn = pa.nodes[pj];
+            if (pn.A1.in != pn.in_dim || !pn.sum_bias.empty()) once = false;
+            for (int c = 0; c < pn.in_dim && once; ++c) {
+                const int pc = pa.conn[pn.in_off + c];
+                if (pc < 0 || pc >= (int)owner.size() || ++reads[pc] > 1) { once = false; break; }
+                const int ci = owner[pc];
+                if (parent_of[ci] < 0) {
+                    parent_of[ci] = pj;
+                    kids[pj].push_back(ci);
+                } else if (parent_of[ci] != pj) {
+                    once = false;
+                }
+            }
+        }
+        for (int r : reads) once = once && r == 1;
+        for (int ci = 0; ci < nc && once; ++ci) once = parent_of[ci] >= 0 && ch.nodes[ci].A2.out == ch.nodes[ci].out_dim;
+        if (!once) {
+            refuse("an overlapping or partial field: every child column must be read exactly once, and all of a child's columns by one parent");
+            continue;
+        }
+        size_t lo = ~(size_t)0, hi = 0;
+        for (auto& k : kids) {
+            lo = std::min(lo, k.size());
+            hi = std::max(hi, k.size());
+        }
+        if (lo != 2 || hi != 2) {
+            refuse((lo == hi ? std::to_string(lo) : std::to_string(lo) + " to " + std::to_string(hi)) + " children per parent, not exactly two");
+            continue;
+        }
+        int p_max = 0;
+        bool plain = true;
+        for (auto& pn : pa.nodes) {
+            p_max = std::max(p_max, pn.A1.out);
+            plain = plain && !rem_tile(pn.A1.out);
+        }
+        const int mtp = (p_max + 15) / 16;
+        if (!plain || mtp > kMaxMT) {
+            refuse("a parent's first affine of " + std::to_string(p_max) + " outputs is not on plain 16-row tiles (its last tile holds 1 to 4 rows), or needs more than 4 tiles");
+            continue;
+        }
+        const HostStage& hc = shapes[l];
+        const int today4 = 2 * (hc.pack_out ? 4 * (hc.mto - 1) + 1 : 4 * hc.mto);
+        if (4 * mtp > today4) {
+            refuse("a parent's " + std::to_string(mtp) + " tiles are more than the " + std::to_string(today4) + " quarter blocks its two children store today");
+            continue;
+        }
+        bool id_pow = true;
+        for (auto& cn : ch.nodes) id_pow = id_pow && cn.funcs.size() == 2 && cn.funcs[0].kind == E_IDENTITY && cn.funcs[1].kind == E_ABS_POW;
+        if (!id_pow) {
+            refuse("the child must expand with exactly (identity, |x|^p)");
+            continue;
+        }
+        if (!(hc.kind == 0 && hc.rem4 && hc.mt1 == 3 && hc.mt2 == 3 && hc.kb1 == 3 && hc.pk_kbi == 1 && hc.pack_in != 0x7fffffff && mtp == 4) || opt.no_rem4) {
+            refuse("no pair sweep is built for this child (built: 3 K-blocks with the slot-major packed block at position 1, three tiles of z with a 4x4 remainder tile, four tiles per parent)");
+            continue;
+        }
+        ch.fold_pairs.clear();
+        ch.fold_bias.clear();
+        for (int pj = 0; pj < np; ++pj) {
+            FNode& pn = pa.nodes[pj];
+            const int P = pn.A1.out;
+            LinkFold lf = fold_link(ch, pa, pj, owner, col0, kids[pj]);
+            ch.fold_pairs.push_back(kids[pj][0]);
+            ch.fold_pairs.push_back(kids[pj][1]);
+            ch.fold_bias.push_back(std::move(lf.bias));
+            pn.kids = kids[pj];
+            pn.sum_bias.assign(P, -0.0);
+            for (int ci : kids[pj]) {
+                FNode& cn = ch.nodes[ci];
+                Aff f;
+                f.in = cn.A2.in;
+                f.out = P;
+                f.a.assign(f.in, 0.0);
+                f.W = std::move(lf.W[ci]);
+                f.b.assign(P, 0.0);
+                cn.A2 = std::move(f);
+                cn.out_dim = P;
+            }
+            pn.A1.a.clear();
+            pn.A1.W.clear();
+            pn.A1.b.clear();
+        }
+        ch.out_w = 0;
+        for (auto& pn : pa.nodes) ch.out_w += pn.A1.out;
+        pa.sum_in = true;
+        pa.pair_in = true;
+        auto issued = [](const HostStage& h) { return "issued: " + std::to_string(h.mfma16_tile) + " x 16x16x4 + " + std::to_string(h.mfma4_tile) + " x 4x4x1"; };
+        note = link + " pair-folded; with the link as the flow gives it stage " + std::to_string(l) + " " + issued(hc) + " and this stage " + issued(shapes[l + 1]);
+        parents.push_back((int)l + 1);
+    }
+    return parents;
+}
+
 namespace {
 
 inline int q_of_row(int i) { return 4 * (i & 3) + (i >> 2); }
@@ -494,6 +625,14 @@
                 if (st.sum_in) {
                     const HostStage& below = stages[stages.size() - 2];
                     if (below.kind != 0 || below.pack_out || below.mto != hs.mt1) fail(HG_ERR_FORMAT, "internal: hoisted link over a layer of another layout");
+                    if (st.pair_in) {
+                        if (below.fold_pairs.size() != (size_t)2 * n) fail(HG_ERR_FORMAT, "internal: pair-folded link without its pair list");
+                        for (int mt = 0; mt < hs.mt1; ++mt) {
+                            K.src.push_back(ni * hs.mt1 + mt);
+                            K.nk.push_back(1);
+                            for (int qq = 0; qq < 16; ++qq) K.kpos.emplace_back();
+                        }
+                    } else
                     for (int ci : nd.kids)
                         for (int mt = 0; mt < hs.mt1; ++mt) {
                             K.src.push_back(ci * below.mto + mt);
@@ -646,7 +785,10 @@
                 const int r1 = hs.p_max - 16 * (hs.mt1 - 1), r2 = hs.s_max - 16 * (hs.mt2 - 1);
                 hs.rem4 = si >= 1 && hs.has_exp && n > 4 && hs.mt1 == hs.mt2 && (hs.mt1 == 2 || hs.mt1 == 3) && r1 >= 1 && r1 <= 4 &&
                           r2 >= 1 && r2 <= 4 && !opt.no_rem4 && !st.sum_in;
-                if (hs.rem4) {
+                const bool fold_out = !st.fold_pairs.empty();
+                hs.rem1 = fold_out && si >= 2 && n > 4 && (hs.mt1 == 2 || hs.mt1 == 3) && r1 >= 1 && r1 <= 4 && !opt.no_rem4;
+                if (fold_out && (hs.rem4 || !hs.rem1)) fail(HG_ERR_FORMAT, "internal: pair-folded stage without a first-affine remainder tile");
+                if (hs.rem4 || hs.rem1) {
                     auto to4x4 = [](float* blk) {
                         float old[256];
                         std::copy(blk, blk + 256, old);
@@ -659,7 +801,7 @@
                         float* wnode = hs.afrag.data() + (size_t)ni * hs.node_blocks * 256;
                         for (int kb = 0; kb < hs.kb1; ++kb) to4x4(wnode + ((size_t)kb * hs.mt1 + hs.mt1 - 1) * 256);
                         float* w2 = wnode + (size_t)hs.kb1 * hs.mt1 * 256;
-                        for (int b2 = 0; b2 < hs.mt1 * hs.nf; ++b2) to4x4(w2 + ((size_t)b2 * hs.mt2 + hs.mt2 - 1) * 256);
+                        for (int b2 = 0; b2 < hs.mt1 * hs.nf && hs.rem4; ++b2) to4x4(w2 + ((size_t)b2 * hs.mt2 + hs.mt2 - 1) * 256);
                     }
                 }
             }
@@ -699,6 +841,20 @@
                     }
                 }
             hs.nb_out = hs.pack_out ? n * (hs.mto - 1) + n / 4 : n * hs.mto;
+            if (!st.fold_pairs.empty()) {
+                const int np = (int)st.fold_pairs.size() / 2;
+                hs.fold_pairs = st.fold_pairs;
+                hs.fold_pair_bias.assign((size_t)np * hs.mto * 16, 0.f);
+                for (int pj = 0; pj < np; ++pj)
+                    for (int mt = 0; mt < hs.mto; ++mt)
+                        for (int gg = 0; gg < 4; ++gg)
+                            for (int r = 0; r < 4; ++r) {
+                                const int fo = 16 * mt + 4 * r + gg;
+                                if (fo < (int)st.fold_bias[pj].size()) hs.fold_pair_bias[((size_t)pj * hs.mto + mt) * 16 + gg * 4 + r] = (float)st.fold_bias[pj][fo];
+                            }
+                hs.nb_out = np * hs.mto;
+            }
+            hs.fold_parent = st.pair_in;
             prev_packed = hs.pack_out;
             prev_blk.swap(cur_blk);
             prev_q.swap(cur_q);
@@ -710,15 +866,22 @@
                 const int rem = (hs.rem4 || front_rem) ? 1 : 0;
                 hs.mfma16_tile = hs.ks1_tile * (hs.mt1 - rem) + (hs.has_exp ? hs.ks2_tile * (hs.mt2 - rem) : 0);
                 hs.mfma4_tile = rem ? hs.ks1_tile + hs.ks2_tile : 0;
+                if (hs.rem1) {
+                    hs.mfma16_tile = hs.ks1_tile * (hs.mt1 - 1) + hs.ks2_tile * hs.mt2;
+                    hs.mfma4_tile = hs.ks1_tile;
+                }
             }
             padded_flops += (hs.mfma16_tile * 2048 + hs.mfma4_tile * 512) / 16;
             std::ostringstream os;
             os << "fused stage " << si << (hs.rem4 ? (hs.pack_out ? " (4x4 remainder tiles, packed four to a block)" : " (4x4 remainder tiles)") : "") << ": " << hs.n_nodes << " nodes, K-blocks " << hs.kb1 << ", tiles " << hs.mt1 << "x" << hs.mt2
-               << (hs.sum_in ? " (first affine folded into the layer below's second, plain 16-row tiles only: z = bias + the tiles of " + std::to_string(hs.n_kids) + " children)" : "")
+               << (hs.sum_in && !hs.fold_parent ? " (first affine folded into the layer below's second, plain 16-row tiles only: z = bias + the tiles of " + std::to_string(hs.n_kids) + " children)" : "")
+               << (hs.fold_parent ? " (first affine run by the pair sweep of the stage below: z = the ONE tile set it stored per node)" : "")
+               << (hs.rem1 ? " (pair sweep: 4x4 remainder tile in the first affine; the second affine is the stage above's first folded in, on plain tiles; both children of a node of the stage above in ONE visit, z of that node stored once: " +
+                                 std::to_string(hs.fold_pairs.size() / 2) + " x " + std::to_string(hs.mto) + " blocks)" : "")
                << ", " << hs.mfma_per_tile << " MFMA/tile (issued: " << hs.mfma16_tile << " x 16x16x4 + " << hs.mfma4_tile << " x 4x4x1), " << hs.afrag.size() * 4 / 1024
                << " KiB weights, out " << hs.nb_out << " blocks/tile";
             hs.name = os.str();
-            if (st.sum_in && opt.pair) plan_pairs(st, hs);
+            if (st.sum_in && opt.pair && !st.pair_in) plan_pairs(st, hs);
         }
         plan_slot_major();
         fuse01 = can_fuse01();
@@ -1306,7 +1469,7 @@
         for (size_t si = 0; si + 1 < stages.size(); ++si) {
             HostStage& pr = stages[si];
             HostStage& co = stages[si + 1];
-            if (!pr.pack_out || co.kind != 0 || !co.rem4 || co.kb1 != 3 || co.mt1 != co.mt2 || (co.mt1 != 2 && co.mt1 != 3)) continue;
+            if (!pr.pack_out || co.kind != 0 || !(co.rem4 ? co.mt1 == co.mt2 : co.rem1) || co.kb1 != 3 || (co.mt1 != 2 && co.mt1 != 3)) continue;
             const int base = pr.n_nodes * (pr.mto - 1);
             int pk = -1;
             bool ok = true;
@@ -1352,7 +1515,7 @@
         int act_blocks = 0, e_blocks = 0;
         while (b > (fuse01 ? 2 : 1) && ns - b < opt.tail_max) {
             const HostStage& s = stages[b - 1];
-            if (s.kind != 0 || s.from_x || s.rem4 || s.pack_out || s.pk_kbi >= 0 || s.pack_in != INT32_MAX || s.nf > kMaxFuncs) break;
+            if (s.kind != 0 || s.from_x || s.rem4 || s.rem1 || s.pack_out || s.pk_kbi >= 0 || s.pack_in != INT32_MAX || s.nf > kMaxFuncs) break;
             if (s.has_exp && s.mt1 * s.nf > 8) break;
             const int waves = s.n_nodes * (s.has_exp ? std::max(s.mt1, s.mt2) : s.mt1);
             if (waves > 16) break;
@@ -1390,7 +1553,7 @@
             std::vector<std::vector<int32_t>> members(kMaxTail), tabs(kMaxTail);
             while (k >= 4 && b > (fuse01 ? 2 : 1) && last + 1 - b < kMaxTail) {
                 const HostStage& s = stages[b - 1];
-                if (s.kind != 0 || s.from_x || s.rem4 || s.pack_out || s.pk_kbi >= 0 || s.pack_in != INT32_MAX || s.nf > kMaxFuncs ||
+                if (s.kind != 0 || s.from_x || s.rem4 || s.rem1 || s.pack_out || s.pk_kbi >= 0 || s.pack_in != INT32_MAX || s.nf > kMaxFuncs ||
                     s.n_nodes % k)
                     break;
                 if (s.has_exp && s.mt1 * s.nf > 8) break;
@@ -1719,21 +1882,41 @@
     }
     if (why_not) why_not->clear();
     int64_t given = -1;
+    std::vector<FStage> plain;
+    auto count_given = [&]() {
+        if (given >= 0 || plain.empty()) return;
+        try {
+            FusedOptions o = opt;
+            o.hoist = false;
+            o.fold01 = false;
+            o.fold01_pack = false;
+            given = Planner(root, std::move(plain), o).padded_flops;
+        } catch (const Error&) {
+        }
+        plain.clear();
+    };
     if (opt.hoist) {
-        std::vector<FStage> plain = stages;
-        if (!hoist_first_affines(stages, opt).empty()) {
-            try {
-                FusedOptions o = opt;
-                o.hoist = false;
-                o.fold01 = false;
-                o.fold01_pack = false;
-                given = Planner(root, std::move(plain), o).padded_flops;
-            } catch (const Error&) {
-            }
+        plain = stages;
+        if (!hoist_first_affines(stages, opt).empty()) count_given();
+    }
+    std::vector<std::string> pair_notes;
+    if (opt.pair_fold && opt.hoist) {
+        try {
+            FusedOptions o = opt;
+            o.fold01 = false;
+            o.fold01_pack = false;
+            o.pair = false;
+            std::vector<FStage> copy = stages;
+            const Planner shapes(root, std::move(copy), o);
+            if (!fold_pair_links(stages, shapes.stages, opt, pair_notes).empty()) count_given();
+        } catch (const Error&) {
+            pair_notes.clear();
         }
     }
     try {
         Planner p(root, std::move(stages), opt);
+        for (size_t i = 0; i < pair_notes.size() && i < p.stages.size(); ++i)
+            if (!pair_notes[i].empty()) p.stages[i].name += "  [" + pair_notes[i] + "]";
         p.padded_flops_given = given >= 0 ? given : p.padded_flops - p.fold01_flops;
         return std::make_unique<const FusedPlan>(std::move(static_cast<FusedPlan&>(p)));
     } catch (const Error& e) {
diff --git a/pyfaceanalysis_amd/csrc/hg_fused_plan.hpp b/pyfaceanalysis_amd/csrc/hg_fused_plan.hpp
--- a/pyfaceanalysis_amd/csrc/hg_fused_plan.hpp
+++ b/pyfaceanalysis_amd/csrc/hg_fused_plan.hpp
@@ -39,6 +39,7 @@
     bool fold01 = false;
     bool fold01_pack = false;
     bool pair = false;
+    bool pair_fold = false;
     int pair_min_wgs = 512;
     static FusedOptions from_env() {
         FusedOptions o;
@@ -111,6 +112,10 @@
     std::vector<int32_t> pair_kids;
     std::vector<int32_t> kb1tab_pre;
     std::vector<float> bias_pre;
+    bool rem1 = false;
+    std::vector<int32_t> fold_pairs;
+    std::vector<float> fold_pair_bias;
+    bool fold_parent = false;
 };
 
 struct FusedPlan {
diff --git a/pyfaceanalysis_amd/csrc/hg_fused_stages.hpp b/pyfaceanalysis_amd/csrc/hg_fused_stages.hpp
--- a/pyfaceanalysis_amd/csrc/hg_fused_stages.hpp
+++ b/pyfaceanalysis_amd/csrc/hg_fused_stages.hpp
@@ -34,11 +34,16 @@
     std::vector<FNode> nodes;
     int out_w = 0;
     bool sum_in = false;
+    std::vector<int32_t> fold_pairs;
+    std::vector<std::vector<double>> fold_bias;
+    bool pair_in = false;
 };
 
 bool build_stages(const TNode& root, std::vector<FStage>& stages, std::string& why, const FusedOptions& opt);
 
 std::vector<int> hoist_first_affines(std::vector<FStage>& stages, const FusedOptions& opt);
 
+std::vector<int> fold_pair_links(std::vector<FStage>& stages, const std::vector<HostStage>& shapes, const FusedOptions& opt, std::vector<std::string>& notes);
+
 }
 }
```

Measured after the change: 10.23 million sub-images/s (median of 6 runs). Within noise of the previous version (+0.4%).
